# tmtlakmal/acme

Hardware: AMD Instinct MI355X
Metric: learner transitions/sec (sample+step) at batch 512, 1/2/4/8 MI355X (higher is better)
Workload: dtype f32 (2xf16 split planes, 3 MFMA terms); 1 GPU; dqn_nature_cnn_prioritized_replay (BASELINE configs[1]); global_batch=512, batch_per_gpu=512, replay_slots=1000000, replay_slots_per_gpu=1000000, obs=uint8[84,84,4], num_actions=18, sampler=prioritized(alpha=0.6), IS beta=0.2, prefetch_size=4, parallelism=dp1

## Files before the change

acme_amd/_lib.py:

```python

from __future__ import annotations

import ctypes
import os
import threading

import torch

_HERE = os.path.dirname(os.path.abspath(__file__))
LIB_PATH = os.environ.get("ACME_LIB_PATH") or os.path.join(_HERE, "libacme_hip.so")

ACME_OK = 0
ACME_ERR_INVALID = -1
ACME_ERR_HIP = -2
ACME_ERR_EMPTY = -3
ACME_ERR_OOM = -4

SEMANTICS_TF = 0
SEMANTICS_JAX = 1

MATMUL_F32 = 0
MATMUL_X6 = 1

MAX_FIELDS = 16
# ... 148 lines not shown
    "acme_set_matmul_engine": (c_i32, [c_i32]),
    "acme_matmul_engine": (c_i32, []),
    "acme_dense_forward": (c_i32, [c_vp, c_i64, c_i64, c_vp, c_vp, c_i64, c_i32, c_vp, c_vp]),
    "acme_dense_forward_staged": (c_i32, [c_vp, c_i64, c_i64, c_vp, c_vp, c_i64, c_i32, c_vp,
                                          c_i32, c_i32, c_i32, c_vp]),
    "acme_replay_create": (c_i32, [ctypes.POINTER(ReplayConfig), ctypes.POINTER(c_vp)]),
    "acme_replay_destroy": (c_i32, [c_vp]),
    "acme_replay_insert": (c_i32, [c_vp, ctypes.POINTER(c_vp), c_i64, c_vp, c_i32, c_vp, c_vp]),
    "acme_replay_stage_capacity": (c_i64, [c_vp]),
    "acme_replay_stage": (c_i32, [c_vp, c_i64, ctypes.POINTER(c_vp)]),
    "acme_replay_commit": (c_i32, [c_vp, c_i64, c_vp, c_vp, c_vp]),
    "acme_replay_sync_inserts": (c_i32, [c_vp]),
    "acme_host_register": (c_i32, [c_vp, c_i64]),
    "acme_event_create": (c_i32, [ctypes.POINTER(c_vp)]),
    "acme_event_destroy": (c_i32, [c_vp]),
    "acme_event_record": (c_i32, [c_vp, c_vp]),
    "acme_stream_wait_event": (c_i32, [c_vp, c_vp]),
    "acme_event_query": (c_i32, [c_vp]),
    "acme_event_synchronize": (c_i32, [c_vp]),
    "acme_host_unregister": (c_i32, [c_vp]),
    "acme_nstep_writer_create": (c_i32, [c_vp, c_i32, c_f32, c_i64, c_i64, c_i64, c_vp]),
    "acme_nstep_writer_destroy": (c_i32, [c_vp]),
    "acme_nstep_writer_start": (c_i32, [c_vp, c_vp]),
    "acme_nstep_writer_add": (c_i32, [c_vp, c_vp, c_f32, c_f32, c_vp, c_i32, c_f64]),
    "acme_nstep_writer_flush": (c_i32, [c_vp]),
    "acme_nstep_writer_reset": (c_i32, [c_vp]),
    "acme_nstep_writer_pending": (c_i64, [c_vp]),
    "acme_replay_fill_synthetic": (c_i32, [c_vp, c_i64, c_i32, c_i32, c_u64, c_vp]),
    "acme_replay_sample": (c_i32, [c_vp, c_i64, c_u64, c_vp, c_vp, c_vp, c_vp, c_vp, c_vp]),
    "acme_replay_gather": (c_i32, [c_vp, c_vp, c_i64, ctypes.POINTER(c_vp), c_vp]),
    "acme_replay_total": (c_i32, [c_vp, c_vp, c_vp]),
    "acme_replay_sample_share": (c_i32, [c_vp, c_i64, c_u64, c_f64, c_vp, c_vp, c_vp, c_vp, c_vp,
                                         ctypes.POINTER(c_vp), c_vp]),
    "acme_replay_sample_share_frames": (c_i32, [c_vp, c_i64, c_u64, c_f64, c_vp, c_vp, c_vp, c_vp,
                                                c_vp, ctypes.POINTER(c_vp), c_vp, c_vp]),
    "acme_replay_sample_gather": (c_i32, [c_vp, c_i64, c_u64, c_vp, c_vp, c_vp, c_vp, c_vp,
                                          ctypes.POINTER(c_vp), c_vp]),
    "acme_replay_sample_gather_frames": (c_i32, [c_vp, c_i64, c_u64, c_vp, c_vp, c_vp, c_vp,
                                                 c_vp, ctypes.POINTER(c_vp), c_vp, c_vp]),
    "acme_replay_pipe_open": (c_i32, [c_vp, ctypes.POINTER(c_i32)]),
    "acme_replay_pipe_close": (c_i32, [c_vp, c_i32]),
    "acme_replay_pipe_flush": (c_i32, [c_vp, c_i32]),
    "acme_replay_sample_gather_pipe": (c_i32, [c_vp, c_i32, c_i64, c_u64, c_vp, c_vp, c_vp, c_vp,
                                               c_vp, ctypes.POINTER(c_vp), c_vp]),
    "acme_r2d2_priorities": (c_i32, [c_vp, c_i32, c_i32, ctypes.c_double, c_vp, c_vp]),
    "acme_r2d2_importance_weights": (c_i32, [c_vp, c_i32, c_i64, ctypes.c_double, c_vp, c_vp]),
    "acme_frames_expand": (c_i32, [c_vp, c_i64, c_i64, c_i32, c_vp, c_i64, c_vp, c_vp]),
    "acme_replay_update_priorities": (c_i32, [c_vp, c_vp, c_vp, c_i64, c_vp]),
    "acme_replay_update_priorities_gated": (c_i32, [c_vp, c_vp, c_vp, c_i64, c_vp, c_vp]),
    "acme_replay_size": (c_i64, [c_vp]),
    "acme_replay_capacity": (c_i64, [c_vp]),
    "acme_replay_debug_leaves": (c_i32, [c_vp, ctypes.POINTER(c_vp), ctypes.POINTER(c_vp),
                                         ctypes.POINTER(c_vp)]),
    "acme_replay_storage": (c_i32, [c_vp, c_i32, ctypes.POINTER(c_vp)]),
    "acme_replay_inserted": (c_i64, [c_vp]),
    "acme_replay_restore": (c_i32, [c_vp, c_i64, c_vp]),
    "acme_dqn_create": (c_i32, [ctypes.POINTER(DQNConfig), ctypes.POINTER(c_vp)]),
    "acme_dqn_destroy": (c_i32, [c_vp]),
    "acme_dqn_num_params": (c_i64, [c_vp]),
    "acme_dqn_flat_size": (c_i64, [c_vp]),
    "acme_dqn_num_tensors": (c_i32, [c_vp]),
    "acme_dqn_tensor_info": (c_i32, [c_vp, c_i32, ctypes.POINTER(c_i64), ctypes.POINTER(c_i64),
                                     ctypes.POINTER(c_i32), ctypes.POINTER(c_i64),
                                     ctypes.POINTER(ctypes.c_char_p)]),
    "acme_dqn_bind": (c_i32, [c_vp, c_vp, c_vp, c_vp, c_vp, c_vp]),
    "acme_dqn_params_changed": (c_i32, [c_vp]),
    "acme_dqn_plane_overflow": (c_i32, [c_vp, ctypes.POINTER(c_i32), c_i32]),
    "acme_dqn_skipped_steps": (c_i64, [c_vp]),
    "acme_dqn_guard_state": (c_i32, [c_vp, ctypes.POINTER(c_i64)]),
    "acme_dqn_verdict_timeouts": (c_i32, [c_vp, ctypes.POINTER(c_i64)]),
    "acme_dqn_set_applied_steps": (c_i32, [c_vp, c_i64]),
    "acme_dqn_skip_word": (c_i32, [c_vp, ctypes.POINTER(c_vp)]),
    "acme_dqn_set_reissue": (c_i32, [c_vp, c_i32]),
    "acme_dqn_verdicts_issued": (c_i64, [c_vp]),
    "acme_dqn_step_verdict": (c_i32, [c_vp, c_i64, ctypes.POINTER(c_i32)]),
    "acme_dqn_set_data_parallel_gate": (c_i32, [c_vp, c_i32]),
    "acme_dqn_dense_grads_ready": (c_i32, [c_vp, c_vp]),
    "acme_dqn_dp_init": (c_i32, [c_vp, c_vp, c_i32]),
    "acme_dqn_dp_step": (c_i32, [c_vp, ctypes.POINTER(TransitionBatch), ctypes.POINTER(DQNOutputs),
                                 c_vp]),
    "acme_nccl_get_unique_id": (c_i32, [c_vp]),
    "acme_nccl_comm_init": (c_i32, [c_vp, c_i32, c_i32, ctypes.POINTER(c_vp)]),
    "acme_nccl_comm_destroy": (c_i32, [c_vp]),
    "acme_dqn_scale_state": (c_i32, [c_vp, c_vp, c_i32, ctypes.POINTER(c_i32)]),
    "acme_dqn_set_scale_state": (c_i32, [c_vp, c_vp, c_i32]),
    "acme_dqn_forward_backward": (c_i32, [c_vp, ctypes.POINTER(TransitionBatch),
                                          ctypes.POINTER(DQNOutputs), c_vp]),
    "acme_dqn_apply": (c_i32, [c_vp, c_vp]),
    "acme_dqn_forward_backward_stage": (c_i32, [c_vp, ctypes.POINTER(TransitionBatch),
                                                ctypes.POINTER(DQNOutputs), c_i32, c_vp]),
    "acme_dqn_grad_split": (c_i32, [c_vp, ctypes.POINTER(c_i64)]),
    "acme_dqn_step": (c_i32, [c_vp, ctypes.POINTER(TransitionBatch), ctypes.POINTER(DQNOutputs),
                              c_vp]),
    "acme_dqn_step_update": (c_i32, [c_vp, ctypes.POINTER(TransitionBatch),
                                     ctypes.POINTER(DQNOutputs), c_vp, c_vp, c_vp, c_vp]),
    "acme_dqn_q_values": (c_i32, [c_vp, c_vp, c_i64, c_i32, c_vp, c_vp]),
    "acme_dqn_num_steps": (c_i64, [c_vp]),
    "acme_dqn_debug_buffer": (c_i32, [c_vp, ctypes.c_char_p, ctypes.POINTER(c_vp),
                                      ctypes.POINTER(c_i64)]),
    "acme_dqn_set_num_steps": (c_i32, [c_vp, c_i64]),
    "acme_min_f64": (c_i32, [c_vp, c_i64, c_vp, c_vp]),
    "acme_r2d2_create": (c_i32, [ctypes.POINTER(R2D2Config), ctypes.POINTER(c_vp)]),
    "acme_r2d2_destroy": (c_i32, [c_vp]),
    "acme_r2d2_flat_size": (c_i64, [c_vp]),
    "acme_r2d2_num_tensors": (c_i32, [c_vp]),
    "acme_r2d2_tensor_info": (c_i32, [c_vp, c_i32, ctypes.POINTER(c_i64), ctypes.POINTER(c_i64),
                                      ctypes.POINTER(c_i32), ctypes.POINTER(c_i64),
                                      ctypes.POINTER(ctypes.c_char_p)]),
    "acme_r2d2_bind": (c_i32, [c_vp, c_vp, c_vp, c_vp, c_vp, c_vp]),
    "acme_r2d2_step": (c_i32, [c_vp, ctypes.POINTER(SequenceBatch), c_vp,
                               ctypes.POINTER(R2D2Outputs), c_vp]),
    "acme_r2d2_params_changed": (c_i32, [c_vp]),
    "acme_r2d2_scale_state": (c_i32, [c_vp, c_vp, c_i32, ctypes.POINTER(c_i32)]),
    "acme_r2d2_set_scale_state": (c_i32, [c_vp, c_vp, c_i32]),
    "acme_r2d2_skipped_steps": (c_i64, [c_vp]),
    "acme_r2d2_guard_state": (c_i32, [c_vp, ctypes.POINTER(c_i64)]),
    "acme_r2d2_skip_word": (c_vp, [c_vp]),
    "acme_r2d2_set_applied_steps": (c_i32, [c_vp, c_i64]),
    "acme_r2d2_num_steps": (c_i64, [c_vp]),
    "acme_r2d2_set_num_steps": (c_i32, [c_vp, c_i64]),
    "acme_r2d2_set_lstm_unroll": (c_i32, [c_vp, c_i32]),
    "acme_r2d2_debug_buffer": (c_i32, [c_vp, ctypes.c_char_p, ctypes.POINTER(c_vp),
                                       ctypes.POINTER(c_i64)]),
# ... 206 lines not shown
```

acme_amd/csrc/common.h:

```cpp
#pragma once

#include <hip/hip_runtime.h>

#include <cstdarg>
#include <cstdint>
#include <cstdio>

#include "../../include/acme_hip.h"

namespace acme {

void set_error(const char* fmt, ...);

int tune_variant(const char* key);
void tune_set(const char* key, int value);
int tune_generation();

hipError_t make_order_event(hipEvent_t* ev);

#define ACME_HIP_TRY(expr)                                                   \
  do {                                                                       \
    hipError_t _e = (expr);                                                  \
    if (_e != hipSuccess) {                                                  \
      ::acme::set_error("%s failed: %s (%s:%d)", #expr, hipGetErrorString(_e), \
                        __FILE__, __LINE__);                                 \
      return ACME_ERR_HIP;                                                   \
    }                                                                        \
  } while (0)

#define ACME_CHECK_ARG(cond, ...)                                            \
  do {                                                                       \
    if (!(cond)) {                                                           \
      ::acme::set_error(__VA_ARGS__);                                        \
      return ACME_ERR_INVALID;                                               \
    }                                                                        \
  } while (0)

#define ACME_LAUNCH_CHECK()                                                  \
  do {                                                                       \
    hipError_t _e = hipGetLastError();                                       \
    if (_e != hipSuccess) {                                                  \
      ::acme::set_error("kernel launch failed: %s (%s:%d)",                  \
                        hipGetErrorString(_e), __FILE__, __LINE__);          \
      return ACME_ERR_HIP;                                                   \
    }                                                                        \
  } while (0)

static inline hipStream_t as_stream(void* s) {
  return reinterpret_cast<hipStream_t>(s);
}

static inline int64_t ceil_div(int64_t a, int64_t b) { return (a + b - 1) / b; }

constexpr int kWave = 64;

__device__ __forceinline__ float wave_sum(float v) {
#pragma unroll
  for (int o = 32; o > 0; o >>= 1) v += __shfl_xor(v, o, 64);
  return v;
}
__device__ __forceinline__ float wave_max(float v) {
#pragma unroll
  for (int o = 32; o > 0; o >>= 1) v = fmaxf(v, __shfl_xor(v, o, 64));
  return v;
}

}
// ... 1 lines not shown
```

acme_amd/csrc/common.hip:

```cpp
#include "common.h"

#include <cstring>
#include <mutex>
#include <string>
#include <utility>
#include <vector>

namespace acme {

static thread_local char g_last_error[1024] = "";

void set_error(const char* fmt, ...) {
  va_list ap;
  va_start(ap, fmt);
  vsnprintf(g_last_error, sizeof(g_last_error), fmt, ap);
  va_end(ap);
}

namespace {
std::mutex g_tune_mu;
std::vector<std::pair<std::string, int>> g_tune;
int g_tune_gen = 0;
}

int tune_generation() {
  std::lock_guard<std::mutex> lock(g_tune_mu);
  return g_tune_gen;
}

int tune_variant(const char* key) {
  std::lock_guard<std::mutex> lock(g_tune_mu);
  for (auto& kv : g_tune)
    if (kv.first == key) return kv.second;
  const char* v = getenv((std::string("ACME_V_") + key).c_str());
  const int x = v ? atoi(v) : 0;
  g_tune.emplace_back(key, x);
  return x;
}

void tune_set(const char* key, int value) {
  std::lock_guard<std::mutex> lock(g_tune_mu);
  ++g_tune_gen;
  for (auto& kv : g_tune)
    if (kv.first == key) {
      kv.second = value;
      return;
    }
  g_tune.emplace_back(key, value);
}

namespace gemm {

static int g_engine = -1;

bool use_x6() {
  if (g_engine < 0) {
    const char* e = getenv("ACME_MATMUL");
    g_engine = (e && strcmp(e, "f32") == 0) ? ACME_MATMUL_F32 : ACME_MATMUL_X6;
  }
  return g_engine == ACME_MATMUL_X6;
}

}

hipError_t make_order_event(hipEvent_t* ev) {
  return hipEventCreateWithFlags(ev, hipEventDisableTiming | hipEventDisableSystemFence);
}

}

extern "C" {

int acme_set_matmul_engine(int32_t engine) {
  ACME_CHECK_ARG(engine == ACME_MATMUL_F32 || engine == ACME_MATMUL_X6, "unknown matmul engine %d",
                 engine);
  acme::gemm::g_engine = engine;
  return ACME_OK;
}

int32_t acme_matmul_engine(void) { return acme::gemm::use_x6() ? ACME_MATMUL_X6 : ACME_MATMUL_F32; }

const char* acme_last_error(void) { return acme::g_last_error; }

int acme_tune_set(const char* key, int32_t value) {
  ACME_CHECK_ARG(key, "null key");
  acme::tune_set(key, value);
  return ACME_OK;
}
// ... 47 lines not shown
```

acme_amd/csrc/dqn.hip:

```cpp
#include <hip/hip_runtime.h>

#include <algorithm>
#include <cmath>
#include <cstring>
#include <string>
#include <vector>

#include "common.h"
#include "conv.h"
#include "rescale.h"
#include "conv_p3.h"
#include "gemm.h"
#include "gemm_p3.h"
#include "gemm_x6.h"
#include "kernels.h"
#include "launch.h"
#include "learner_common.h"
#include "plane_guard.h"
#include "profiler.h"
#include "rccl_dyn.h"
#include "torso.h"

using namespace acme;
using namespace acme::conv;
using acme::gemm::launch_gemm;

namespace {

using torso::G1;
constexpr int kFlat = torso::kFlat;
constexpr int kHidden = 512;
constexpr int kObsBytes = 84 * 84 * 4;

struct Layer {
  int in = 0, out = 0;
  int w = -1, b = -1;
  bool relu = true;
};

}

struct acme_dqn : PlaneGuard {
  acme_dqn_config cfg;
  std::vector<Tensor> tensors;
  int64_t flat = 0, logical = 0;
  float *params = nullptr, *target = nullptr, *grads = nullptr, *m = nullptr, *v = nullptr;
  int64_t num_steps = 0;
  int t_c1w = -1, t_c1b, t_c2w, t_c2b, t_c3w, t_c3b, t_fcw, t_fcb, t_vw, t_vb, t_aw, t_ab;
  std::vector<Layer> layers;
  std::vector<void*> allocs;
  float *x1 = nullptr, *x2 = nullptr, *x3 = nullptr, *hid = nullptr;
  float *t1 = nullptr, *t2 = nullptr, *t3 = nullptr, *thid = nullptr;
  std::vector<float*> mlp_act, mlp_tact, mlp_dz;
  float *q_on = nullptr, *q_tg = nullptr;
  float *dzh = nullptr, *dz3 = nullptr, *dz2 = nullptr, *dz1 = nullptr;
  float* slab = nullptr;
  int64_t slab_floats = 0;
  bool stamps_on = false;
  uint64_t* stamps = nullptr;
  float* g = nullptr;
  int32_t* a_cache = nullptr;
  float* loss_tmp = nullptr;
  float* td_tmp = nullptr;
  double* prio_tmp = nullptr;
  bool p3_capable = false;
  bool planes_stale = true;
  bool last_p3 = false;
  uint16_t *wpl = nullptr, *tpl = nullptr;
  bool calibrating = false;
  int64_t fwd_batch = 0;
  uint16_t* frames = nullptr;
  torso::Frames cur_frames{nullptr};
  hipStream_t side = nullptr;
  hipEvent_t ev[4] = {nullptr, nullptr, nullptr, nullptr};
  float* slab2 = nullptr;
  bool fused_step = false;
  acme_replay* upd_replay = nullptr;
  const uint64_t* upd_keys = nullptr;
  hipEvent_t upd_after = nullptr;
  const double* upd_prio = nullptr;
  int upd_n = 0;
  bool slabs_pending = false;
  torso::WgradSlab wslabs[3];
  float* side_slab = nullptr;
  float* tslab = nullptr;
  bool target_dirty = true;
  torso::Plane x1p{}, x2p{}, x3p{}, t1p{}, t2p{}, t3p{}, dzhp{}, dz3p{}, dz2p{}, dz1p{};
  LossArgs pending_la{};
  bool loss_pending = false;
  bool head_deferred = false;
  int head_splits = 0;
  int64_t loss_nparts = 0;
  hipEvent_t ev_dense = nullptr;
  hipEvent_t dense_ev = nullptr;
  bool dense_on_side = false;
  void* dp_comm = nullptr;
  int dp_world = 0;
  hipStream_t dp_stream = nullptr;
  hipEvent_t dp_ev[4] = {nullptr, nullptr, nullptr, nullptr};
  double* dp_gmin = nullptr;
  double* loss_part = nullptr;
  bool single_stream = false;
  bool single_role = false;
  bool bk32 = false;
  bool frames_u8 = true;
  int64_t seq = 0;
  uint32_t* host_verdicts = nullptr;
  uint32_t verdict_seq = 0;
  bool sticky = false;
  bool dp_gate = false;
  int64_t dp_gate_index = -1;
  bool step_rescaled = false;
};

namespace {

enum {
  kScX1, kScX2, kScX3, kScT1, kScT2, kScT3, kScDzh, kScDz3, kScDz2, kScDz1,
  kScTransient,
  kScParams = kScTransient, kScTarget,
  kScCount
};
constexpr int64_t kParamAmaxPeriod = 8;
constexpr int kVerdictRing = 64;

int add_tensor(acme_dqn* l, const std::string& name, std::initializer_list<int64_t> shape) {
  const int t = acme::add_tensor<acme_dqn>(l, name, shape);
  l->logical += l->tensors[t].numel;
  return t;
}

inline torso::Plane WP(const acme_dqn* l, uint16_t* base, int t) {
  return torso::Plane{base + l->tensors[t].offset, l->flat,
                      l->scales + (base == l->tpl ? kScTarget : kScParams)};
}
int convert_frames(acme_dqn* l, const void* obs_a, const void* obs_b, int split, int rows,
                   hipStream_t st) {
  ACME_PROF("frames_f16", st, 0.0, 3.0 * (double)rows * kObsBytes);
  return launch_frames_f16(static_cast<const uint8_t*>(obs_a), static_cast<const uint8_t*>(obs_b),
                           split, rows, kObsBytes, l->frames, st);
}
bool use_p3(const acme_dqn* l) { return l->p3_capable && gemm::use_x6(); }
Gate step_gate(const acme_dqn* l) {
  Gate q;
  q.g = l->guard;
  q.par = (int)(l->seq & 1);
  if (l->dp_gate) q.dp = l->grads + l->dp_gate_index;
  return q;
}
hipStream_t side_stream(const acme_dqn* l) { return prof::enabled() ? nullptr : l->side; }

constexpr int kFcFwdSplits = 8;
constexpr int kHeadFwdSplits = 16;
constexpr int kHeadBwdSplits = 8;

int64_t slab_floats_needed(int B, int A) {
  return std::max<int64_t>({torso::wgrad_slab_floats(), (int64_t)kFcFwdSplits * 2 * B * 2 * kHidden,
// ... 117 lines not shown
    ACME_GEMM("mlp_fwd", 64, 64, 2, 2, 16, 1, p, 1);
  }
  return ACME_OK;
}

int mlp_forward(acme_dqn* l, const float* prm, const void* obs_a, const void* obs_b, int split,
                int rows, std::vector<float*>& act, float* q, hipStream_t st) {
  const int nl = (int)l->layers.size();
  for (int i = 0; i < nl; ++i) {
    const Layer& L = l->layers[i];
    float* y = i == nl - 1 ? q : act[i];
    int rc;
    if (i == 0) {
      rc = l->cfg.obs_dtype == ACME_OBS_U8_SCALED
               ? mlp_layer<InU8>(l, prm, L, obs_a, obs_b, split, rows, y, st)
               : mlp_layer<InF32>(l, prm, L, obs_a, obs_b, split, rows, y, st);
    } else {
      rc = mlp_layer<InF32>(l, prm, L, act[i - 1], act[i - 1], rows, rows, y, st);
    }
    if (rc != ACME_OK) return rc;
  }
  return ACME_OK;
}

RescaleJob step_rescale_job(acme_dqn* l, bool defer_r) {
  RescaleJob j;
  j.s = l->scales;
  j.nt = j.n = kScTransient;
  j.overflow = l->overflow;
  j.skip_lo = kScT1;
  j.skip_hi = kScT3 + 1;
  j.defer_r = defer_r ? 1 : 0;
  j.rg.g = l->guard;
  j.rg.mode = kRgStep;
  j.rg.gate = step_gate(l);
  j.rg.host_skipped = l->host_skipped;
  j.rg.host_verdicts = l->host_verdicts;
  j.rg.seq = l->verdict_seq++;
  j.rg.sticky = l->sticky ? 1 : 0;
  return j;
}

int priority_update_tail(void* ctx, hipStream_t st) {
  acme_dqn* l = static_cast<acme_dqn*>(ctx);
  acme_replay* r = l->upd_replay;
  if (!r || !l->upd_prio) return ACME_OK;
  l->upd_replay = nullptr;
  if (l->upd_after) ACME_HIP_TRY(hipStreamWaitEvent(st, l->upd_after, 0));
  const RescaleJob job = step_rescale_job(l, true);
  const int rc =
      replay_update_priorities_gated(r, l->upd_keys, l->upd_prio, l->upd_n, step_gate(l), st, &job);
  if (rc == ACME_OK) l->step_rescaled = true;
  return rc;
}

int nature_backward(acme_dqn* l, const void* o_tm1, int B, hipStream_t st_main,
                    bool join_dense) {
  hipStream_t st = st_main;
  const float* prm = l->params;
  float* gr = l->grads;
  const int A = l->cfg.num_actions;
  const bool p3 = use_p3(l);
  int rc;
  bool loss_sum = false;
  const LossArgs la = l->pending_la;
  if (p3 && l->loss_pending && l->head_deferred) {
    l->loss_pending = l->head_deferred = false;
    loss_sum = true;
    l->loss_nparts = B;
    ACME_PROF("head_loss_dz", st, 0.0, 4.0 * (double)2 * B * 2 * kHidden * (l->head_splits + 1));
    rc = launch_dqn_head_loss_dz(la, l->slab, l->head_splits, kHidden, P(l, prm, l->t_fcb),
                                 P(l, prm, l->t_vw), P(l, prm, l->t_vb), P(l, prm, l->t_aw),
                                 P(l, prm, l->t_ab), l->hid, l->dzhp.p, l->dzhp.stride,
                                 l->dzhp.sc, st);
    if (rc != ACME_OK) return rc;
  } else if (p3 && l->loss_pending) {
    l->loss_pending = false;
    loss_sum = la.loss_part != nullptr;
    l->loss_nparts = dqn_loss_head_dz_blocks(B, kHidden);
    ACME_PROF("loss_head_dz", st, 0.0, 0.0);
    rc = launch_dqn_loss_head_dz(la, l->hid, kHidden, P(l, prm, l->t_vw),
                                 P(l, prm, l->t_aw), l->dzhp.p, l->dzhp.stride, l->dzhp.sc, st);
    if (rc != ACME_OK) return rc;
  } else {
    ACME_PROF("head_dz", st, 0.0, 0.0);
    rc = p3 ? launch_head_dz_planes(l->hid, l->g, l->a_cache, B, kHidden, A, P(l, prm, l->t_vw),
                                    P(l, prm, l->t_aw), l->dzhp.p, l->dzhp.stride, l->dzhp.sc, st)
            : launch_duel_head_dz(l->hid, l->g, l->a_cache, B, kHidden, A, P(l, prm, l->t_vw),
                                  P(l, prm, l->t_aw), l->dzh, st);
    if (rc != ACME_OK) return rc;
  }
  const bool fork = p3 && side_stream(l);
  float* hslab = fork ? l->side_slab : l->slab;
  if (fork) {
    ACME_HIP_TRY(hipEventRecord(l->ev[2], st_main));
    ACME_HIP_TRY(hipStreamWaitEvent(l->side, l->ev[2], 0));
    st = l->side;
  }
  if (p3 && l->upd_replay && !l->calibrating) {
    l->upd_prio = la.prio;
    l->upd_n = B;
  }
  const bool sum_in_scatter = loss_sum;
  {
    DuelHeadWgrad p;
    p.M = 2 * kHidden; p.N = A + 1; p.K = B; p.k_chunk = chunk_for(B, kHeadBwdSplits);
// ... 93 lines not shown
        ACME_GEMM("mlp_dgrad", 64, 64, 2, 2, 16, 1, p, 1);
      } else {
        DenseDgrad<false> p;
        p.M = B; p.N = L.in; p.K = L.out; p.k_chunk = L.out;
        p.dz = dz; p.w = P(l, prm, L.w); p.xprev = l->mlp_act[i - 1]; p.ldx = L.in;
        p.dx = l->mlp_dz[i - 1];
        ACME_GEMM("mlp_dgrad", 64, 64, 2, 2, 16, 1, p, 1);
      }
    }
  }
  return ACME_OK;
}

int sync_planes(acme_dqn* l, hipStream_t st) {
  if (!l->p3_capable || !l->planes_stale) return ACME_OK;
  int rc = launch_split_planes(l->params, l->flat, l->wpl, l->flat, l->scales + kScParams, st,
                               l->overflow, 1);
  if (rc == ACME_OK)
    rc = launch_split_planes(l->target, l->flat, l->tpl, l->flat, l->scales + kScTarget, st,
                             l->overflow, 1);
  if (rc == ACME_OK) l->planes_stale = false;
  return rc;
}

int reset_scales(acme_dqn* l) {
  return scales_init(l, kScCount, [l](int i) {
    return i >= kScT1 && i <= kScT3 ? &l->guard->tt
           : i >= kScTransient     ? &l->guard->prm
                                   : &l->guard->on;
  });
}

}

extern "C" {

int acme_dqn_create(const acme_dqn_config* cfg, acme_dqn** out) {
  ACME_CHECK_ARG(cfg && out, "null argument");
  ACME_CHECK_ARG(cfg->num_actions >= 1 && cfg->num_actions <= 63, "num_actions must be in [1, 63]");
  ACME_CHECK_ARG(cfg->max_batch >= 1 && cfg->max_batch <= 65536, "max_batch must be in [1, 65536]");
  ACME_CHECK_ARG(cfg->network == ACME_NET_NATURE_DQN || cfg->network == ACME_NET_MLP,
                 "unknown network kind %d", cfg->network);
  ACME_CHECK_ARG(cfg->obs_dtype == ACME_OBS_U8_SCALED || cfg->obs_dtype == ACME_OBS_F32,
                 "unknown observation dtype %d", cfg->obs_dtype);
  ACME_CHECK_ARG(cfg->huber_loss_parameter >= 0.f, "quadratic_linear_boundary must be >= 0.");
  ACME_CHECK_ARG(cfg->target_update_period >= 1, "target_update_period must be >= 1");
  ACME_CHECK_ARG(cfg->semantics == ACME_SEMANTICS_TF || cfg->semantics == ACME_SEMANTICS_JAX,
                 "unknown learner semantics %d", cfg->semantics);
  acme_dqn* l = new acme_dqn();
  l->cfg = *cfg;
  l->single_stream = tune_variant("SIDE") == 1;
  l->single_role = tune_variant("WSN") == 1;
  l->bk32 = tune_variant("BK32") == 1;
  l->stamps_on = tune_variant("STAMPS") == 1;
  const int A = cfg->num_actions;
  const int B = cfg->max_batch;
  int rc = ACME_OK;
  auto fail = [&](int code) {
    acme_dqn_destroy(l);
    return code;
  };
  if ((rc = guard_create(l)) != ACME_OK) return fail(rc);
  if (hipHostMalloc(reinterpret_cast<void**>(&l->host_verdicts), kVerdictRing * sizeof(uint32_t),
                    hipHostMallocCoherent | hipHostMallocMapped) != hipSuccess)
    return fail((set_error("step guard allocation failed"), ACME_ERR_HIP));
  for (int i = 0; i < kVerdictRing; ++i) l->host_verdicts[i] = 0xFFFFFFFFu;
  if (cfg->network == ACME_NET_NATURE_DQN) {
    l->t_c1w = add_tensor(l, "atari_torso/conv2_d/w", {8, 8, 4, 32});
    l->t_c1b = add_tensor(l, "atari_torso/conv2_d/b", {32});
    l->t_c2w = add_tensor(l, "atari_torso/conv2_d_1/w", {4, 4, 32, 64});
    l->t_c2b = add_tensor(l, "atari_torso/conv2_d_1/b", {64});
    l->t_c3w = add_tensor(l, "atari_torso/conv2_d_2/w", {3, 3, 64, 64});
    l->t_c3b = add_tensor(l, "atari_torso/conv2_d_2/b", {64});
    l->t_fcw = add_tensor(l, "duelling_q_network/hidden/w", {kFlat, 2 * kHidden});
    l->t_fcb = add_tensor(l, "duelling_q_network/hidden/b", {2 * kHidden});
    l->t_vw = add_tensor(l, "duelling_q_network/mlp/linear_1/w", {kHidden, 1});
    l->t_vb = add_tensor(l, "duelling_q_network/mlp/linear_1/b", {1});
    l->t_aw = add_tensor(l, "duelling_q_network/mlp_1/linear_1/w", {kHidden, A});
    l->t_ab = add_tensor(l, "duelling_q_network/mlp_1/linear_1/b", {A});
    const int R2 = 2 * B;
    if ((rc = dev_alloc(l, &l->x1, (int64_t)R2 * G1::OPIX * G1::CO)) ||
        (rc = dev_alloc(l, &l->x2, (int64_t)R2 * kFlat)) ||
        (rc = dev_alloc(l, &l->x3, (int64_t)R2 * kFlat)) ||
        (rc = dev_alloc(l, &l->hid, (int64_t)R2 * 2 * kHidden)) ||
        (rc = dev_alloc(l, &l->t1, (int64_t)B * G1::OPIX * G1::CO)) ||
        (rc = dev_alloc(l, &l->t2, (int64_t)B * kFlat)) ||
        (rc = dev_alloc(l, &l->t3, (int64_t)B * kFlat)) ||
        (rc = dev_alloc(l, &l->thid, (int64_t)B * 2 * kHidden)) ||
        (rc = dev_alloc(l, &l->dzh, (int64_t)B * 2 * kHidden)) ||
        (rc = dev_alloc(l, &l->dz3, (int64_t)B * kFlat)) ||
        (rc = dev_alloc(l, &l->dz2, (int64_t)B * kFlat)) ||
        (rc = dev_alloc(l, &l->dz1, (int64_t)B * G1::OPIX * G1::CO)))
      return fail(rc);
    l->slab_floats = slab_floats_needed(B, A);
    if (cfg->obs_dtype == ACME_OBS_U8_SCALED && (int64_t)R2 * kObsBytes * 2 < (int64_t)INT32_MAX) {
      l->p3_capable = true;
      const int64_t fl = l->flat;
      if ((rc = reset_scales(l)) ||
          (rc = dev_alloc(l, &l->wpl, gemm::kPlanes * fl)) ||
          (rc = dev_alloc(l, &l->tpl, gemm::kPlanes * fl)) ||
          (rc = dev_alloc(l, &l->frames, (int64_t)R2 * kObsBytes)) ||
          (rc = plane_alloc(l, &l->x1p, (int64_t)R2 * torso::kX1, kScX1)) ||
          (rc = plane_alloc(l, &l->x2p, (int64_t)R2 * kFlat, kScX2)) ||
          (rc = plane_alloc(l, &l->x3p, (int64_t)R2 * kFlat, kScX3)) ||
          (rc = plane_alloc(l, &l->t1p, (int64_t)B * torso::kX1, kScT1)) ||
          (rc = plane_alloc(l, &l->t2p, (int64_t)B * kFlat, kScT2)) ||
// ... 109 lines not shown
  l->grads = grads;
  l->m = adam_m;
  l->v = adam_v;
  l->planes_stale = true;
  l->scales_ok = false;
  return ACME_OK;
}

int acme_dqn_params_changed(acme_dqn* l) {
  ACME_CHECK_ARG(l, "null learner");
  l->planes_stale = true;
  l->scales_ok = false;
  l->target_dirty = true;
  return ACME_OK;
}

int acme_dqn_scale_state(const acme_dqn* l, float* out, int32_t capacity, int32_t* count) {
  return scale_state(l, out, capacity, count);
}

int acme_dqn_set_scale_state(acme_dqn* l, const float* in, int32_t count) {
  const int rc = set_scale_state(l, in, count);
  if (rc == ACME_OK) l->target_dirty = true;
  return rc;
}

int acme_dqn_plane_overflow(acme_dqn* l, int32_t* overflow, int32_t reset) {
  return plane_overflow(l, overflow, reset);
}

int64_t acme_dqn_skipped_steps(const acme_dqn* l) { return skipped_steps(l); }

int acme_dqn_guard_state(acme_dqn* l, int64_t* out4) {
  ACME_CHECK_ARG(l && out4 && l->guard, "null argument");
  StepGuard g;
  if (int rc = read_guard(l, &g)) return rc;
  out4[0] = g.applied;
  out4[1] = g.skipped;
  out4[2] = g.last;
  out4[3] = g.qv;
  return ACME_OK;
}

int acme_dqn_verdict_timeouts(acme_dqn* l, int64_t* out) {
  ACME_CHECK_ARG(l && out, "null argument");
  *out = 0;
  if (!l->guard) return ACME_OK;
  StepGuard g;
  if (int rc = read_guard(l, &g)) return rc;
  *out = g.vtimeout;
  return ACME_OK;
}

int acme_dqn_set_reissue(acme_dqn* l, int32_t enable) {
  ACME_CHECK_ARG(l, "null learner");
  l->sticky = enable != 0 && l->p3_capable;
  return ACME_OK;
}

int64_t acme_dqn_verdicts_issued(const acme_dqn* l) { return l ? (int64_t)l->verdict_seq : 0; }

int acme_dqn_step_verdict(const acme_dqn* l, int64_t seq, int32_t* state) {
  ACME_CHECK_ARG(l && state && seq >= 0, "bad argument");
  *state = -1;
  if (!l->host_verdicts || seq >= (int64_t)l->verdict_seq) return ACME_OK;
  ACME_CHECK_ARG(seq + kVerdictRing >= (int64_t)l->verdict_seq,
                 "verdict %lld is older than the ring's %d", (long long)seq, kVerdictRing);
  const uint32_t v =
      __atomic_load_n(l->host_verdicts + (seq & (kVerdictRing - 1)), __ATOMIC_ACQUIRE);
  if ((v >> 1) == ((uint32_t)seq & 0x7fffffffu)) *state = (int32_t)(v & 1u);
  return ACME_OK;
}

int acme_dqn_set_applied_steps(acme_dqn* l, int64_t n) {
  ACME_CHECK_ARG(l && l->guard && n >= 0, "bad argument");
  return set_applied(l, n);
}

int acme_dqn_skip_word(const acme_dqn* l, const uint32_t** out) {
  ACME_CHECK_ARG(l && out, "null argument");
  *out = l->p3_capable ? &l->guard->last : nullptr;
  return ACME_OK;
}

int acme_dqn_set_data_parallel_gate(acme_dqn* l, int32_t enable) {
  ACME_CHECK_ARG(l, "null learner");
  if (enable && l->cfg.network == ACME_NET_NATURE_DQN && l->p3_capable) {
    const Tensor& t = l->tensors[l->t_c1b];
    ACME_CHECK_ARG(align64(t.offset + t.numel) > t.offset + t.numel, "no padding word for the gate");
    l->dp_gate_index = t.offset + t.numel;
    l->dp_gate = true;
  } else {
    l->dp_gate = false;
  }
  return ACME_OK;
}

int64_t acme_dqn_num_steps(const acme_dqn* l) { return l ? l->num_steps : 0; }
int acme_dqn_set_num_steps(acme_dqn* l, int64_t n) {
  ACME_CHECK_ARG(l && n >= 0, "bad argument");
  l->num_steps = n;
  return ACME_OK;
}

int acme_dqn_debug_buffer(const acme_dqn* l, const char* name, const float** out,
                          int64_t* count) {
// ... 85 lines not shown
constexpr int kCalibrationPasses = 4;
static int calibrate_scales(acme_dqn* l, const acme_transition_batch* batch, hipStream_t st) {
  acme_transition_batch cb = *batch;
  cb.global_min_probability = nullptr;
  l->calibrating = true;
  int rc = ACME_OK;
  for (int pass = 0; pass < kCalibrationPasses && rc == ACME_OK; ++pass) {
    rc = forward_backward_stage(l, &cb, nullptr, 2, st, false);
    if (rc == ACME_OK) rc = forward_backward_stage(l, &cb, nullptr, 3, st, false);
    if (rc == ACME_OK) rc = forward_backward_stage(l, &cb, nullptr, 1, st, false);
    if (rc == ACME_OK)
      rc = launch_plane_rescale(l->scales, kScTransient, kScTransient, -1, -1, l->overflow, st);
  }
  l->calibrating = false;
  if (rc != ACME_OK) return rc;
  return calibration_done(l, st);
}

static int forward_backward_stage(acme_dqn* l, const acme_transition_batch* batch,
                                  const acme_dqn_outputs* out, int32_t stage, void* stream,
                                  bool join_dense) {
  ACME_CHECK_ARG(l && batch && l->params, "null argument or unbound learner");
  ACME_CHECK_ARG(stage >= 0 && stage <= 4, "stage must be 0, 1, 2, 3 or 4");
  ACME_CHECK_ARG(batch->o_tm1 && batch->a_tm1 && batch->r_t && batch->d_t && batch->o_t &&
                     batch->probabilities,
                 "transition batch has null fields");
  ACME_CHECK_ARG(batch->batch >= 1 && batch->batch <= l->cfg.max_batch,
                 "batch %lld outside [1, max_batch=%d]", (long long)batch->batch, l->cfg.max_batch);
  hipStream_t st = as_stream(stream);
  const int B = (int)batch->batch;
  const bool nature = l->cfg.network == ACME_NET_NATURE_DQN;
  if (stage == 1) {
    if (!nature) return ACME_OK;
    if (use_p3(l)) {
      torso::Grads g{Pm(l, l->grads, l->t_c1w), Pm(l, l->grads, l->t_c1b),
                     Pm(l, l->grads, l->t_c2w), Pm(l, l->grads, l->t_c2b),
                     Pm(l, l->grads, l->t_c3w), Pm(l, l->grads, l->t_c3b)};
      torso::PWeights w{WP(l, l->wpl, l->t_c1w), WP(l, l->wpl, l->t_c2w),
                        WP(l, l->wpl, l->t_c3w), P(l, l->params, l->t_c1b),
                        P(l, l->params, l->t_c2b), P(l, l->params, l->t_c3b)};
      torso::Side sd;
      sd.single_role = l->single_role;
      sd.bk32 = l->bk32;
      sd.conv1_single = true;
      if (side_stream(l)) {
        sd.side = l->side;
        sd.slab = l->side_slab;
        for (int i = 0; i < 3; ++i) sd.e[i] = l->ev[i];
      }
      l->slabs_pending = false;
      if (l->upd_replay && l->upd_prio && !l->calibrating) {
        sd.tail = priority_update_tail;
        sd.tail_ctx = l;
      }
      if (l->fused_step && !l->calibrating && l->slab2) {
        sd.slab = l->side_slab;
        sd.slab2 = l->slab2;
        sd.defer = l->wslabs;
        l->slabs_pending = true;
      }
      int rc = torso::backward_p3(w, g, l->cur_frames, B,
                                  torso::PActs{l->x1p, l->x2p, l->x3p}, l->dz3p, l->dz2p, l->dz1p,
                                  l->slab, st, sd);
      if (rc == ACME_OK && l->dp_gate && !l->calibrating) {
        Gate local = step_gate(l);
        local.dp = nullptr;
        rc = launch_gate_publish(local, l->grads + l->dp_gate_index, st, l->scales,
                                 kScTransient, kScT1, kScT3 + 1);
      }
      return rc;
    }
    torso::Grads g{Pm(l, l->grads, l->t_c1w), Pm(l, l->grads, l->t_c1b), Pm(l, l->grads, l->t_c2w),
                   Pm(l, l->grads, l->t_c2b), Pm(l, l->grads, l->t_c3w), Pm(l, l->grads, l->t_c3b)};
    return torso::backward(torso_weights(l, l->params), g,
                           l->cfg.obs_dtype == ACME_OBS_U8_SCALED, batch->o_tm1, B,
                           torso::Acts{l->x1, l->x2, l->x3}, l->dz3, l->dz2, l->dz1, l->slab, st);
  }
  const int A = l->cfg.num_actions;
  int rc;
  if (stage == 3 || stage == 4) {
    ACME_CHECK_ARG(l->fwd_batch == (int64_t)B, "stage %d needs the stage-2 forward of this batch",
                   stage);
    l->fwd_batch = 0;
    return loss_and_dense_backward(l, batch, out, st, join_dense && stage == 3);
  }
  l->last_p3 = nature && use_p3(l);
  if (l->last_p3) {
    const bool u8 = !batch->obs_f16 && l->frames_u8 &&
                    ((reinterpret_cast<uintptr_t>(batch->o_tm1) |
                      reinterpret_cast<uintptr_t>(batch->o_t)) & 15) == 0;
    const bool quiet =
        !l->planes_stale && l->scales_ok && (batch->obs_f16 || u8) && !l->calibrating;
    if ((rc = sync_planes(l, st)) != ACME_OK) return rc;
    if (!l->scales_ok && !l->calibrating && (rc = calibrate_scales(l, batch, st)) != ACME_OK)
      return rc;
    l->last_p3 = true;
    hipStream_t tst = st;
    hipStream_t side = side_stream(l);
    if (!batch->obs_f16 && !u8 &&
        (rc = convert_frames(l, batch->o_tm1, batch->o_t, B, 2 * B, st)) != ACME_OK)
      return rc;
    const torso::Frames fwd_frames =
        u8 ? torso::Frames{batch->o_tm1, true, batch->o_t, B}
           : torso::Frames{batch->obs_f16 ? static_cast<const void*>(batch->obs_f16)
                                          : static_cast<const void*>(l->frames)};
    l->cur_frames = fwd_frames;
// ... 338 lines not shown
```

acme_amd/csrc/gemm_p3.h:

```cpp
#pragma once

#include <hip/hip_runtime.h>

#include <cstdint>
#include <type_traits>

#include "gemm.h"
#include "gemm_x6.h"

namespace acme {
namespace gemm {

struct BlockPlace {
  int m0, n0, z;
};
template <int BM, int BN>
__device__ __forceinline__ BlockPlace place_block(int M, int N, int n_major) {
  const int tiles = gridDim.x;
  const int total = tiles * gridDim.z;
  const int orig = blockIdx.x + tiles * blockIdx.z;
  const int xcd = orig & 7, q = total >> 3, r = total & 7;
  const int L = (xcd < r ? xcd * (q + 1) : r * (q + 1) + (xcd - r) * q) + (orig >> 3);
  const int z = L / tiles, t = L - z * tiles;
  const int tiles_m = (M + BM - 1) / BM, tiles_n = (N + BN - 1) / BN;
  int mt, nt;
  if (n_major) {
    nt = t / tiles_m;
    mt = t - nt * tiles_m;
  } else {
    mt = t / tiles_n;
    nt = t - mt * tiles_n;
  }
  return BlockPlace{mt * BM, nt * BN, z};
}
template <class P>
__device__ __forceinline__ P z_select_at(const P& p, int z) {
  if constexpr (HasZClass<P>::value) return p.for_z(z);
  else return p;
}

using u32x4 = __attribute__((ext_vector_type(4))) uint32_t;
using i16x4 = __attribute__((ext_vector_type(4))) short;
using f16x8 = __attribute__((ext_vector_type(8))) _Float16;

__device__ __forceinline__ u32x4 zero_u4() { return u32x4{0u, 0u, 0u, 0u}; }

constexpr uint32_t kOOB = 0x80000000u;

constexpr int kPlanes = 2;

constexpr int kAmaxSlots = 64;
struct PScale {
  float w, r, wi, rl;
  uint32_t* flag;
  uint32_t pad1[26];
  struct Slot {
    uint32_t v;
    uint32_t pad[31];
  } slot[kAmaxSlots];
};
static_assert(sizeof(PScale) == 128 * (1 + kAmaxSlots), "one 128-B line per amax slot");
__device__ __forceinline__ float read_scale(const PScale* s) { return s ? s->r : 1.f; }

struct PlaneSrc {
  const uint16_t* p;
  int64_t stride;
  int32_t bytes;
  const PScale* sc = nullptr;
};
__device__ __forceinline__ __amdgpu_buffer_rsrc_t plane_rsrc(const PlaneSrc& s, int pl) {
  return __builtin_amdgcn_make_buffer_rsrc(const_cast<uint16_t*>(s.p + pl * s.stride), (short)0,
                                           s.bytes, 0x00020000);
}
__device__ __forceinline__ float result_scale(const PlaneSrc& a, const PlaneSrc& b) {
  return read_scale(a.sc) * read_scale(b.sc);
}

__device__ __forceinline__ void split2_bits(float y, uint16_t& h, uint16_t& l) {
  const _Float16 hb = (_Float16)y;
  const _Float16 lb = (_Float16)(y - (float)hb);
  h = __builtin_bit_cast(uint16_t, hb);
  l = __builtin_bit_cast(uint16_t, lb);
}
__device__ __forceinline__ float f16_bits_to_f32(uint16_t b) {
  return (float)__builtin_bit_cast(_Float16, b);
}
// ... 375 lines not shown
                                                  int wave, int wm, int wn, int lane, int split,
                                                  f32x16 (&acc)[MT][NTL], f32x16 (&cs)[NCS],
                                                  bool do_colsum,
                                                  const typename EpiPre<P>::type* pre = nullptr) {
    static_assert(HasStore8<P>::value, "plane problems store 8 columns at a time");
    const int r = lane & 31, h = lane >> 5;
    typename EpiPre<P>::type pl{};
    if constexpr (EpiPre<P>::has) pl = pre ? *pre : p.pre(n0 + wn * TN + epi_col(lane));
    constexpr int PITCH = TN + 4;
    float* cw = reinterpret_cast<float*>(smem) + wave * 32 * PITCH;
    constexpr int CHUNKS = 32 * TN / 8;
    float amx = 0.f;
#pragma unroll
    for (int i = 0; i < MT; ++i) {
#pragma unroll
      for (int j = 0; j < NTL; ++j)
#pragma unroll
        for (int v = 0; v < 16; ++v)
          cw[((v & 3) + 8 * (v >> 2) + 4 * h) * PITCH + j * 32 + r] = acc[i][j][v];
      __syncthreads();
#pragma unroll
      for (int c = lane; c < CHUNKS; c += 64) {
        const int row = c / (TN / 8), col = 8 * (c % (TN / 8));
        const int m = m0 + wm * TM + i * 32 + row;
        const int n = n0 + wn * TN + col;
        const f32x4 lo = *reinterpret_cast<const f32x4*>(cw + row * PITCH + col);
        const f32x4 hi = *reinterpret_cast<const f32x4*>(cw + row * PITCH + col + 4);
        const float v8[8] = {lo[0], lo[1], lo[2], lo[3], hi[0], hi[1], hi[2], hi[3]};
        if constexpr (EpiPre<P>::has) {
          if (m < p.M && n < p.N) amx = amax_max(amx, p.store8p(m, n, v8, split, pl));
        } else {
          if (m < p.M && n < p.N) amx = amax_max(amx, p.store8(m, n, v8, split));
        }
      }
      __syncthreads();
    }
    if constexpr (HasAmax<P>::value) {
      if constexpr (EpiPre<P>::has) amax_commit_pre(p.amax_sc(), amx, pl.w, pl.flag);
      else amax_commit(p.amax_sc(), amx);
    }
    if constexpr (kColSum) {
      if (do_colsum && h == 0) {
#pragma unroll
        for (int j = 0; j < NTL; ++j) {
          const int n = n0 + wn * TN + j * 32 + r;
          if (n < p.N) p.store_colsum(n, cs[j][0], split);
        }
      }
    }
  }
};

template <int BM, int BN, int WM, int WN, int BK, bool DEEP, class P>
__global__ void __launch_bounds__(64 * WM * WN) gemm_p3_kernel(const P p_in, int n_major) {
  using C = P3Core<BM, BN, WM, WN, BK, P>;
  using PA = typename C::PA;
  using PB = typename C::PB;
  constexpr int NT = C::NT, NPA = C::NPA, NPB = C::NPB, STAGE = C::STAGE;
  const BlockPlace bp = place_block<BM, BN>(p_in.M, p_in.N, n_major);
  const P p = z_select_at(p_in, bp.z);
  extern __shared__ __attribute__((aligned(16))) uint8_t smem[];

  const int tid = threadIdx.x;
  const int lane = tid & 63, wave = tid >> 6;
  const int wm = wave / WN, wn = wave % WN;
  const int m0 = bp.m0, n0 = bp.n0;
  const int split = HasZClass<P>::value ? 0 : bp.z;
  const int kbeg = split * p.k_chunk;
  int kend = kbeg + p.k_chunk;
  if (kend > p.K) kend = p.K;
  const int nk = kend > kbeg ? (kend - kbeg + BK - 1) / BK : 0;

  typename P::ARow arow[PA::PER_THREAD];
  typename P::BRow brow[PB::PER_THREAD];
#pragma unroll
  for (int i = 0; i < PA::PER_THREAD; ++i)
    arow[i] = p.a_row(m0 + (PA::owns(tid + i * NT) ? PA::row_of(tid + i * NT) : 0));
#pragma unroll
  for (int i = 0; i < PB::PER_THREAD; ++i)
    brow[i] = p.b_row(n0 + (PB::owns(tid + i * NT) ? PB::row_of(tid + i * NT) : 0));

  __amdgpu_buffer_rsrc_t srcA[NPA], srcB[NPB];
#pragma unroll
  for (int pl = 0; pl < NPA; ++pl) srcA[pl] = plane_rsrc(p.a_src, pl);
#pragma unroll
  for (int pl = 0; pl < NPB; ++pl) srcB[pl] = plane_rsrc(p.b_src, pl);

  constexpr int SETS = DEEP ? 2 : 1;
  u32x4 ra[SETS][PA::PER_THREAD][NPA], rb[SETS][PB::PER_THREAD][NPB];
  auto fetch = [&](auto S, int k0) {
    constexpr int set = decltype(S)::value;
#pragma unroll
    for (int i = 0; i < PA::PER_THREAD; ++i) {
      const int u = tid + i * NT;
      const int kk = PA::kk_of(u);
      const uint32_t off = (PA::owns(u) && k0 + kk < kend) ? p.a_off(arow[i], k0, kk) : kOOB;
#pragma unroll
      for (int pl = 0; pl < NPA; ++pl) {
        ra[set][i][pl] = load_a_unit<P>(srcA[pl], off);
      }
    }
#pragma unroll
    for (int i = 0; i < PB::PER_THREAD; ++i) {
      const int u = tid + i * NT;
      const int kk = PB::kk_of(u);
      const uint32_t off = (PB::owns(u) && k0 + kk < kend) ? p.b_off(brow[i], k0, kk) : kOOB;
#pragma unroll
      for (int pl = 0; pl < NPB; ++pl)
        rb[set][i][pl] =
            __builtin_bit_cast(u32x4, __builtin_amdgcn_raw_buffer_load_b128(srcB[pl], off, 0, 0));
    }
  };
  auto stash = [&](auto S, int buf) {
    constexpr int set = decltype(S)::value;
// ... 23 lines not shown
  acc.zero();
  const bool do_colsum = C::kColSum && m0 == 0 && wm == 0;
  auto compute = [&](int buf) {
    const uint8_t* sa = smem + buf * STAGE;
    C::mma(sa, sa + PA::BYTES, wm, wn, lane, acc, do_colsum);
  };

  using S0 = std::integral_constant<int, 0>;
  using S1 = std::integral_constant<int, 1>;
  if constexpr (DEEP) {
    if (nk > 0) {
      fetch(S0{}, kbeg);
      stash(S0{}, 0);
    }
    if (nk > 1) fetch(S1{}, kbeg + BK);
    __syncthreads();
    auto iter = [&](auto S, int kt) {
      constexpr int set = decltype(S)::value;
      using Other = std::integral_constant<int, set ^ 1>;
      if constexpr (BK == 32) {
        const uint8_t* sa = smem + set * STAGE;
        C::template mma<0, 1>(sa, sa + PA::BYTES, wm, wn, lane, acc, do_colsum);
        stash(Other{}, set ^ 1);
        fetch(S, kbeg + (kt + 2) * BK);
        C::template mma<1, 2>(sa, sa + PA::BYTES, wm, wn, lane, acc, do_colsum);
      } else {
        stash(Other{}, set ^ 1);
        fetch(S, kbeg + (kt + 2) * BK);
        compute(set);
      }
      __syncthreads();
    };
    int kt = 0;
    for (; kt + 1 < nk; kt += 2) {
      iter(S0{}, kt);
      iter(S1{}, kt + 1);
    }
    if (kt < nk) iter(S0{}, kt);
  } else {
    if (nk > 0) {
      fetch(S0{}, kbeg);
      stash(S0{}, 0);
    }
    __syncthreads();
    for (int kt = 0; kt < nk; ++kt) {
      const bool more = kt + 1 < nk;
      if (more) fetch(S0{}, kbeg + (kt + 1) * BK);
      compute(kt & 1);
      if (more) stash(S0{}, (kt + 1) & 1);
      __syncthreads();
    }
  }
  C::epilogue(p, smem, m0, n0, wave, wm, wn, lane, split, acc, do_colsum);
}

template <int BM, int BN, int WM, int WN, int BK, int STAGES, class P>
__global__ void __launch_bounds__(64 * WM * WN) gemm_p3g_kernel(const P p_in, int n_major) {
#if defined(__HIP_DEVICE_COMPILE__)
  using C = P3Core<BM, BN, WM, WN, BK, P>;
  using PA = typename C::PA;
  using PB = typename C::PB;
  constexpr int NW = WM * WN, NPA = C::NPA, NPB = C::NPB, STAGE = C::STAGE;
  constexpr int PWA = (PA::BLOCKS + NW - 1) / NW, PWB = (PB::BLOCKS + NW - 1) / NW;
  static_assert(!AU8<P>::value, "LDS-DMA copies bytes as they are: no uint8 A operand");
  constexpr int D = PWA * NPA + PWB * NPB;
  static_assert(STAGES >= 2 && STAGES <= 4, "2..4 LDS stages");
  static_assert((STAGES - 2) * D <= 63, "vmcnt range");
  const BlockPlace bp = place_block<BM, BN>(p_in.M, p_in.N, n_major);
  const P p = z_select_at(p_in, bp.z);
  extern __shared__ __attribute__((aligned(16))) uint8_t smem[];
  uint8_t* scratch = smem + STAGES * STAGE;

  const int tid = threadIdx.x;
  const int lane = tid & 63, wave = __builtin_amdgcn_readfirstlane(tid >> 6);
  const int wm = wave / WN, wn = wave % WN;
  const int m0 = bp.m0, n0 = bp.n0;
  const int split = HasZClass<P>::value ? 0 : bp.z;
  const int kbeg = split * p.k_chunk;
  int kend = kbeg + p.k_chunk;
  if (kend > p.K) kend = p.K;
  const int nk = kend > kbeg ? (kend - kbeg + BK - 1) / BK : 0;

  typename P::ARow arow[PWA];
  typename P::BRow brow[PWB];
  int akk[PWA], bkk[PWB];
#pragma unroll
  for (int j = 0; j < PWA; ++j) {
    const int b = wave + NW * j;
    const int u = 64 * (b < PA::BLOCKS ? b : 0) + lane;
    arow[j] = p.a_row(m0 + PA::slot_row(u));
    akk[j] = PA::slot_kk(u);
  }
#pragma unroll
  for (int j = 0; j < PWB; ++j) {
    const int b = wave + NW * j;
    const int u = 64 * (b < PB::BLOCKS ? b : 0) + lane;
    brow[j] = p.b_row(n0 + PB::slot_row(u));
    bkk[j] = PB::slot_kk(u);
  }
  __amdgpu_buffer_rsrc_t srcA[NPA], srcB[NPB];
#pragma unroll
  for (int pl = 0; pl < NPA; ++pl) srcA[pl] = plane_rsrc(p.a_src, pl);
#pragma unroll
  for (int pl = 0; pl < NPB; ++pl) srcB[pl] = plane_rsrc(p.b_src, pl);

  typedef __attribute__((address_space(3))) void lds_void;
// ... 208 lines not shown
      C::mma(sa, sa + PA::BYTES, wm, wn, lane, acc, do_colsum);
      rbuf = rbuf == RING - 1 ? 0 : rbuf + 1;
      __syncthreads();
    }
  }
  if constexpr (HasStamps<P>::value)
    if (stamp) st_t2 = __builtin_amdgcn_s_memtime();
  C::epilogue(p, smem, m0, n0, wave, wm, wn, lane, split, acc, do_colsum);
  if constexpr (HasStamps<P>::value) {
    if (stamp) {
      const uint64_t t3 = __builtin_amdgcn_s_memtime(), rt1 = __builtin_amdgcn_s_memrealtime();
      uint64_t* o = p.stamps + 8 * ((int64_t)blockIdx.z * gridDim.x + blockIdx.x);
      o[0] = st_rt0;
      o[1] = rt1;
      o[2] = st_t0;
      o[3] = st_t1;
      o[4] = st_t2;
      o[5] = t3;
    }
  }
}

template <class P>
inline int p3_n_major(const P& p) {
  return (int64_t)p.N * P::B_PLANES > (int64_t)p.M * P::A_PLANES ? 1 : 0;
}

template <class P>
constexpr double p3_peak_tflops() {
  return 2500.0 / (double)p3_nterms<P::A_PLANES, P::B_PLANES>();
}

template <class Kern>
inline hipError_t p3_set_lds(Kern* k, int lds) {
  if (lds <= 65536) return hipSuccess;
  return hipFuncSetAttribute(reinterpret_cast<const void*>(k),
                             hipFuncAttributeMaxDynamicSharedMemorySize, lds);
}

template <int BM, int BN, int WM, int WN, int BK, bool DEEP = true, class P>
inline hipError_t launch_gemm_p3(const P& p, int splits, hipStream_t st) {
  using C = P3Core<BM, BN, WM, WN, BK, P>;
  constexpr int STAGES_BYTES = 2 * C::STAGE;
  constexpr int LDS = STAGES_BYTES > C::EPI_BYTES ? STAGES_BYTES : C::EPI_BYTES;
  static_assert(LDS <= 160 * 1024, "two stages must fit the 160-KiB LDS of a CU");
  static hipError_t attr = p3_set_lds(&gemm_p3_kernel<BM, BN, WM, WN, BK, DEEP, P>, LDS);
  if (attr != hipSuccess) return attr;
  const int tiles = ((p.N + BN - 1) / BN) * ((p.M + BM - 1) / BM);
  hipLaunchKernelGGL((gemm_p3_kernel<BM, BN, WM, WN, BK, DEEP, P>), dim3(tiles, 1, splits),
                     dim3(C::NT), LDS, st, p, p3_n_major(p));
  return hipGetLastError();
}

template <int BM, int BN, int WM, int WN, int BK, bool PIPE = false, class P>
inline hipError_t launch_gemm_p3ws(const P& p, int splits, hipStream_t st) {
  using C = P3Core<BM, BN, WM, WN, BK, P>;
  constexpr int RING_BYTES = 3 * C::STAGE;
  constexpr int LDS = RING_BYTES > C::EPI_BYTES ? RING_BYTES : C::EPI_BYTES;
  static_assert(LDS <= 160 * 1024, "three stages must fit the 160-KiB LDS of a CU");
  static hipError_t attr = p3_set_lds(&gemm_p3ws_kernel<BM, BN, WM, WN, BK, PIPE, P>, LDS);
  if (attr != hipSuccess) return attr;
  const int tiles = ((p.N + BN - 1) / BN) * ((p.M + BM - 1) / BM);
  hipLaunchKernelGGL((gemm_p3ws_kernel<BM, BN, WM, WN, BK, PIPE, P>), dim3(tiles, 1, splits),
                     dim3(2 * C::NT), LDS, st, p, p3_n_major(p));
  return hipGetLastError();
}

template <int BM, int BN, int WM, int WN, int BK, int STAGES, class P>
inline hipError_t launch_gemm_p3g(const P& p, int splits, hipStream_t st) {
  using C = P3Core<BM, BN, WM, WN, BK, P>;
  constexpr int RING = STAGES * C::STAGE + 1024;
  constexpr int LDS = RING > C::EPI_BYTES ? RING : C::EPI_BYTES;
  static_assert(LDS <= 160 * 1024, "the stage ring must fit the 160-KiB LDS of a CU");
  static hipError_t attr = p3_set_lds(&gemm_p3g_kernel<BM, BN, WM, WN, BK, STAGES, P>, LDS);
  if (attr != hipSuccess) return attr;
  const int tiles = ((p.N + BN - 1) / BN) * ((p.M + BM - 1) / BM);
  hipLaunchKernelGGL((gemm_p3g_kernel<BM, BN, WM, WN, BK, STAGES, P>), dim3(tiles, 1, splits),
                     dim3(C::NT), LDS, st, p, p3_n_major(p));
  return hipGetLastError();
}

}
}
```

acme_amd/csrc/replay.hip:

```cpp
#include <hip/hip_runtime.h>

#include <algorithm>
#include <cmath>
#include <cstring>
#include <condition_variable>
#include <mutex>
#include <thread>
#include <vector>

#include "common.h"
#include "detmath.h"
#include "kernels.h"
#include "profiler.h"
#include "rescale.h"

namespace acme {
uint64_t* g_update_stamps = nullptr;
}

using namespace acme;

constexpr int kStageChunks = 4;
constexpr int64_t kStageBytes = 32ll << 20;
constexpr int kMaxReaders = 8;
constexpr int kMaxPipes = 8;

struct acme_replay {
  acme_replay_config cfg;
  int nlevels = 0;
  int64_t level_size[8] = {};
  double* levels[8] = {};
  double* raw_prio = nullptr;
  uint64_t* keys = nullptr;
  int32_t* winner = nullptr;
  uint32_t* upd_done = nullptr;
  int64_t* upd_slots = nullptr;
  int32_t* upd_valid = nullptr;
  int64_t upd_cap = 0;
  uint8_t* fields[ACME_MAX_FIELDS] = {};
  int64_t inserted = 0;
  std::mutex mu;
  hipStream_t side = nullptr;
  hipStream_t upload = nullptr;
  hipEvent_t insert_event = nullptr;
  uint64_t insert_seq = 0;
  int64_t stage_items = 0;
  int64_t stage_off[ACME_MAX_FIELDS + 3] = {};
  uint8_t* stage[kStageChunks] = {};
  uint8_t* stage_dev[kStageChunks] = {};
  hipEvent_t stage_up[kStageChunks] = {};
  hipEvent_t stage_done[kStageChunks] = {};
  bool stage_used[kStageChunks] = {};
  int stage_next = 0;
  int staged = -1;
  int64_t staged_n = 0;
  std::thread::id staged_by;
  std::condition_variable stage_cv;
  struct Reader {
    hipStream_t s;
    hipEvent_t ev;
    uint64_t waited;
    bool dirty;
  } readers[kMaxReaders] = {};
  int nreaders = 0;
  std::mutex order_mu;
  struct Pipe {
    bool open, pending;
    hipEvent_t ev;
    hipStream_t st;
    int64_t batch;
    const int64_t* slots;
    void* out[ACME_MAX_FIELDS];
  } pipes[kMaxPipes] = {};
};

namespace {

__device__ __forceinline__ double wave_scan64(double x) {
  const int lane = threadIdx.x & 63;
#pragma unroll
  for (int d = 1; d < 64; d <<= 1) {
    double y = __shfl_up(x, d, 64);
    if (lane >= d) x = y + x;
  }
  return x;
}

template <int Ctrl>
__device__ __forceinline__ double dpp_f64(double x) {
  const uint64_t u = __builtin_bit_cast(uint64_t, x);
  const int lo = __builtin_amdgcn_mov_dpp((int)(uint32_t)u, Ctrl, 0xf, 0xf, false);
  const int hi = __builtin_amdgcn_mov_dpp((int)(uint32_t)(u >> 32), Ctrl, 0xf, 0xf, false);
  return __builtin_bit_cast(double, ((uint64_t)(uint32_t)hi << 32) | (uint32_t)lo);
}
__device__ __forceinline__ double wave_total64(double x) {
  x = x + dpp_f64<0xB1>(x);
  x = x + dpp_f64<0x4E>(x);
  x = x + dpp_f64<0x141>(x);
  x = x + dpp_f64<0x140>(x);
  const uint64_t u = __builtin_bit_cast(uint64_t, x);
  const int lo = __builtin_amdgcn_ds_swizzle((int)(uint32_t)u, 0x401F);
  const int hi = __builtin_amdgcn_ds_swizzle((int)(uint32_t)(u >> 32), 0x401F);
  x = x + __builtin_bit_cast(double, ((uint64_t)(uint32_t)hi << 32) | (uint32_t)lo);
  const uint64_t v = __builtin_bit_cast(uint64_t, x);
  const uint32_t a0 = __builtin_amdgcn_readlane((int)(uint32_t)v, 31);
  const uint32_t a1 = __builtin_amdgcn_readlane((int)(uint32_t)(v >> 32), 31);
  const uint32_t b0 = __builtin_amdgcn_readlane((int)(uint32_t)v, 63);
  const uint32_t b1 = __builtin_amdgcn_readlane((int)(uint32_t)(v >> 32), 63);
  return __builtin_bit_cast(double, ((uint64_t)a1 << 32) | a0) +
         __builtin_bit_cast(double, ((uint64_t)b1 << 32) | b0);
}

__device__ __forceinline__ int select_child(double v, double s, double t) {
  const uint64_t le = __ballot(s <= t);
  const uint64_t nz = __ballot(v > 0.0);
  int idx = __popcll(le);
  const int last = nz ? 63 - __clzll(nz) : 0;
  if (idx > last) idx = last;
  return idx;
}

constexpr int kTopComputed = 16;
struct TreeView {
  const double* level[8];
  int nlevels;
  int top_nodes = 0;
};

__device__ __forceinline__ double top_entry(const double* const* level, int nlevels,
                                            int top_nodes) {
  const int lane = threadIdx.x & 63;
  if (top_nodes <= 0) return level[nlevels - 1][lane];
  const double* c = level[nlevels - 2];
  double ch[kTopComputed];
#pragma unroll
  for (int g = 0; g < kTopComputed; ++g) ch[g] = g < top_nodes ? c[g * 64 + lane] : 0.0;
  double v = 0.0;
#pragma unroll
  for (int g = 0; g < kTopComputed; ++g) {
    if (g >= top_nodes) break;
    const double t = wave_total64(ch[g]);
    if (lane == g) v = t;
  }
  return v;
}

__device__ __forceinline__ bool draw_prioritized(const TreeView& tree, double u,
                                                 int64_t* slot_out, double* prob_out) {
  const int lane = threadIdx.x & 63;
  int64_t node = 0;
  double t = 0.0, total = 0.0, leaf_value = 0.0;
  const int top = tree.nlevels - 1;
  double ch[kTopComputed];
  for (int l = top; l >= 0; --l) {
    const int64_t base = node * 64;
    double v;
    if (l == top) {
      if (tree.top_nodes > 0) {
        const double* c = tree.level[top - 1];
#pragma unroll
        for (int g = 0; g < kTopComputed; ++g) ch[g] = g < tree.top_nodes ? c[g * 64 + lane] : 0.0;
        v = 0.0;
#pragma unroll
        for (int g = 0; g < kTopComputed; ++g) {
          if (g >= tree.top_nodes) break;
// ... 384 lines not shown
    int shift) {
  const int lane = threadIdx.x & 63;
  const int64_t j = (int64_t)blockIdx.x * (blockDim.x >> 6) + (threadIdx.x >> 6);
  if (j >= count) return;
  int64_t node;
  if (slots) {
    if (valid && !valid[j]) return;
    node = slots[j] >> shift;
  } else {
    node = node_begin + j;
  }
  const double v = child[node * 64 + lane];
  const double s = wave_total64(v);
  if (lane == 63) parent[node] = s;
}

__global__ void prio_resolve_kernel(const uint64_t* __restrict__ upd_keys, int64_t n,
                                    const uint64_t* __restrict__ keys, int64_t capacity,
                                    int64_t* __restrict__ out_slots,
                                    int32_t* __restrict__ valid, int32_t* __restrict__ winner) {
  const int64_t j = (int64_t)blockIdx.x * blockDim.x + threadIdx.x;
  if (j >= n) return;
  const uint64_t k = upd_keys[j];
  const int64_t slot = (int64_t)(k % (uint64_t)capacity);
  const int ok = keys[slot] == k;
  out_slots[j] = slot;
  valid[j] = ok;
  if (ok) atomicMax(&winner[slot], (int32_t)j);
}

__global__ void prio_write_kernel(const double* __restrict__ prios, int64_t n,
                                  const int64_t* __restrict__ slots,
                                  const int32_t* __restrict__ valid,
                                  const int32_t* __restrict__ winner, double alpha,
                                  double* __restrict__ raw_prio, double* __restrict__ leaves,
                                  const Gate gate) {
  const int64_t j = (int64_t)blockIdx.x * blockDim.x + threadIdx.x;
  if (j >= n || !valid[j] || gate_skip(gate)) return;
  const int64_t slot = slots[j];
  if (winner[slot] != (int32_t)j) return;
  const double p = prios[j];
  raw_prio[slot] = p;
  leaves[slot] = det_pow_priority(p, alpha);
}

__global__ void prio_reset_kernel(const int64_t* __restrict__ slots,
                                  const int32_t* __restrict__ valid, int64_t n,
                                  int32_t* __restrict__ winner) {
  const int64_t j = (int64_t)blockIdx.x * blockDim.x + threadIdx.x;
  if (j >= n || !valid[j]) return;
  winner[slots[j]] = -1;
}

constexpr int kFusedUpdateMax = 4096;
constexpr int kFusedUpdateBlocks = 256;
constexpr int kUpdPairs = 32;
struct FusedUpdateArgs {
  const uint64_t* upd_keys;
  const double* prios;
  int n;
  int64_t capacity;
  const uint64_t* keys;
  double alpha;
  double* raw_prio;
  double* level[8];
  int64_t top_nodes;
  int top_computed;
  int nlevels;
  uint32_t* done;
  Gate gate;
  RescaleJob job;
  uint64_t* stamps = nullptr;
};
__device__ __forceinline__ bool wait_verdict_skip(StepGuard* g, uint32_t seq, uint32_t first) {
  __shared__ uint32_t s_v;
  if (threadIdx.x == 0) {
    uint32_t v = first;
    for (int it = 0; it < (1 << 22) && (v >> 1) != (seq & 0x7fffffffu); ++it) {
      __builtin_amdgcn_s_sleep(2);
      v = __hip_atomic_load(&g->vseq, __ATOMIC_RELAXED, __HIP_MEMORY_SCOPE_AGENT);
    }
    const bool got = (v >> 1) == (seq & 0x7fffffffu);
    if (!got) atomicAdd(&g->vtimeout, 1u);
    s_v = got ? (v & 1u) : 1u;
  }
  __syncthreads();
  return s_v != 0u;
}
__device__ __forceinline__ void lds_barrier() {
  __builtin_amdgcn_fence(__ATOMIC_RELEASE, "workgroup", "local");
  __builtin_amdgcn_s_barrier();
  __builtin_amdgcn_fence(__ATOMIC_ACQUIRE, "workgroup", "local");
}
__device__ __forceinline__ void store_shared_level(double* p, double v) {
  __hip_atomic_store(p, v, __ATOMIC_RELAXED, __HIP_MEMORY_SCOPE_AGENT);
}
template <int R>
__global__ void __launch_bounds__(256) prio_update_fused_kernel(FusedUpdateArgs a) {
  static_assert(R * 256 <= kFusedUpdateMax, "update capacity");
  __shared__ int64_t s_slot[R * 256];
  __shared__ int s_len, s_np, s_ovf, s_last;
  __shared__ double s_ch[kUpdPairs][64];
  __shared__ int64_t s_node[kUpdPairs];
  __shared__ int s_lvl[kUpdPairs];
  __shared__ int64_t s_nk[kUpdPairs];
  __shared__ double s_val[kUpdPairs];
  const int first = a.job.s ? 1 : 0;
  auto stamp = [&](int ph) {
    if (a.stamps && threadIdx.x == 0)
      a.stamps[8 * (int64_t)blockIdx.x + ph] = __builtin_amdgcn_s_memrealtime();
  };
  stamp(0);
  if (a.job.s && blockIdx.x == 0) {
    rescale_block(a.job);
    stamp(1);
    return;
  }
  const bool verdict = a.job.s && a.job.rg.g && a.job.rg.mode == kRgStep;
  const int tid = threadIdx.x, nt = blockDim.x;
  const int lane = tid & 63, wave = tid >> 6, nw = nt >> 6;
  const int G = kFusedUpdateBlocks, bid = (int)blockIdx.x - first;
  const int h = a.nlevels >= 2 ? a.nlevels - 2 : 0;
  bool skip = !verdict && gate_skip(a.gate);
  if (tid == 0) s_len = 0;
  __syncthreads();
  uint64_t kv[R];
  double pr[R];
  int64_t sl[R];
  int my_e[R];
#pragma unroll
  for (int i = 0; i < R; ++i) {
    my_e[i] = -1;
    kv[i] = 0;
    pr[i] = 0.0;
    sl[i] = 0;
  }
  if (!skip) {
#pragma unroll
    for (int i = 0; i < R; ++i) {
      if (i * nt >= a.n) break;
      const int j = tid + i * nt;
      const int jc = j < a.n ? j : a.n - 1;
      kv[i] = a.upd_keys[jc];
      pr[i] = a.prios[jc];
    }
#pragma unroll
    for (int i = 0; i < R; ++i) {
      if (i * nt >= a.n) break;
      const int j = tid + i * nt;
      const int64_t slot = (int64_t)(kv[i] % (uint64_t)a.capacity);
      if (j < a.n && (int)((slot >> (6 * h)) % G) == bid) {
        const int e = atomicAdd(&s_len, 1);
        s_slot[e] = slot;
        my_e[i] = e;
        sl[i] = slot;
      }
    }
  }
  __syncthreads();
  stamp(1);
  const int len = s_len;
  if (len > 0) {
    if (tid == 0) {
      s_np = 0;
      s_ovf = 0;
    }
    __syncthreads();
    for (int idx = tid; idx < h * len; idx += nt) {
      const int l = 1 + idx / len, e = idx - (l - 1) * len;
      const int64_t node = s_slot[e] >> (6 * l);
      bool first = true;
      for (int f = 0; f < e && first; ++f) first = (s_slot[f] >> (6 * l)) != node;
      if (!first) continue;
      const int q = atomicAdd(&s_np, 1);
      if (q < kUpdPairs) {
        s_lvl[q] = l;
        s_node[q] = node;
        s_nk[q] = (node << 3) | l;
      } else {
        s_ovf = 1;
      }
    }
    __syncthreads();
    if (tid == 0 && s_np > kUpdPairs) s_np = kUpdPairs;
    __syncthreads();
    stamp(2);
    const int np = s_np;
    const bool pre = !s_ovf;
    uint64_t kt[R];
#pragma unroll
    for (int i = 0; i < R; ++i) {
      if (i * nt >= a.n) break;
      kt[i] = my_e[i] >= 0 ? a.keys[sl[i]] : 0;
    }
    if (pre) {
      for (int q = wave; q < np; q += nw)
        s_ch[q][lane] = a.level[s_lvl[q] - 1][s_node[q] * 64 + lane];
    }
    double leafv[R];
#pragma unroll
    for (int i = 0; i < R; ++i) {
      if (i * nt >= a.n) break;
      leafv[i] = 0.0;
      if (my_e[i] >= 0) leafv[i] = det_pow_priority(pr[i], a.alpha);
    }
#pragma unroll
    for (int i = 0; i < R; ++i) {
      if (i * nt >= a.n) break;
      if (my_e[i] >= 0)
        s_slot[my_e[i]] = (sl[i] << 13) | ((kt[i] == kv[i] ? 1 : 0) << 12) | (tid + i * nt);
    }
    __syncthreads();
    stamp(4);
    uint32_t vfirst = 0;
    if (verdict && tid == 0)
      vfirst = __hip_atomic_load(&a.job.rg.g->vseq, __ATOMIC_RELAXED, __HIP_MEMORY_SCOPE_AGENT);
    bool winv[R];
#pragma unroll
    for (int i = 0; i < R; ++i) winv[i] = false;
#pragma unroll
    for (int i = 0; i < R; ++i) {
      if (i * nt >= a.n) break;
      const int e = my_e[i];
      bool win = e >= 0 && kt[i] == kv[i];
      const int j = tid + i * nt;
      const int64_t me = (sl[i] << 1) | 1;
#pragma unroll 4
      for (int f = 0; f < len; ++f) {
        const int64_t x = s_slot[f];
        if ((x >> 12) == me && (int)(x & 4095) > j) win = false;
      }
      winv[i] = win;
    }
    if (pre) {
#pragma unroll
      for (int i = 0; i < R; ++i) {
        if (i * nt >= a.n) break;
        if (!winv[i]) continue;
        const int64_t k1 = ((sl[i] >> 6) << 3) | 1;
#pragma unroll 4
        for (int q = 0; q < np; ++q)
          if (s_nk[q] == k1) s_ch[q][sl[i] & 63] = leafv[i];
      }
    }
    lds_barrier();
    if (pre) {
      for (int l = 1; l <= h; ++l) {
        for (int q = wave; q < np; q += nw) {
          if (s_lvl[q] != l) continue;
          const double v = wave_total64(s_ch[q][lane]);
          if (lane == 63) s_val[q] = v;
        }
        lds_barrier();
        if (tid < np && s_lvl[tid] == l) {
          const int64_t kp = ((s_node[tid] >> 6) << 3) | (l + 1);
#pragma unroll 4
          for (int q = 0; q < np; ++q)
            if (s_nk[q] == kp) s_ch[q][s_node[tid] & 63] = s_val[tid];
        }
        lds_barrier();
      }
    }
    stamp(7);
    if (verdict) skip = wait_verdict_skip(a.job.rg.g, a.job.rg.seq, vfirst);
    stamp(3);
    if (!skip) {
#pragma unroll
      for (int i = 0; i < R; ++i) {
        if (i * nt >= a.n) break;
        if (!winv[i]) continue;
        a.raw_prio[sl[i]] = pr[i];
        if (h == 0 && !a.top_computed) store_shared_level(a.level[0] + sl[i], leafv[i]);
        else a.level[0][sl[i]] = leafv[i];
      }
      if (pre) {
        for (int q = tid; q < np; q += nt) {
          const int l = s_lvl[q];
          if (l == h && !a.top_computed) store_shared_level(a.level[l] + s_node[q], s_val[q]);
          else a.level[l][s_node[q]] = s_val[q];
        }
      } else {
        __syncthreads();
        for (int l = 1; l <= h; ++l) {
          for (int e = wave; e < len; e += nw) {
            const int64_t node = (s_slot[e] >> 13) >> (6 * l);
            const double v = wave_total64(a.level[l - 1][node * 64 + lane]);
            if (lane == 63) {
              if (l == h && !a.top_computed) store_shared_level(a.level[l] + node, v);
              else a.level[l][node] = v;
            }
          }
          __syncthreads();
        }
      }
      stamp(5);
    }
  }
  stamp(6);
  if (a.nlevels < 2 || a.top_computed) return;
  __builtin_amdgcn_fence(__ATOMIC_RELEASE, "agent");
  __syncthreads();
  if (tid == 0)
    s_last = __hip_atomic_fetch_add(a.done, 1u, __ATOMIC_ACQ_REL, __HIP_MEMORY_SCOPE_AGENT) ==
             (uint32_t)(G - 1);
  __syncthreads();
  if (!s_last) return;
  __builtin_amdgcn_fence(__ATOMIC_ACQUIRE, "agent");
  const int top = a.nlevels - 1;
  for (int64_t node = wave; node < a.top_nodes; node += nw) {
    const double c = __hip_atomic_load(a.level[top - 1] + node * 64 + lane, __ATOMIC_RELAXED,
                                       __HIP_MEMORY_SCOPE_AGENT);
    const double v = wave_total64(c);
    if (lane == 63) a.level[top][node] = v;
  }
  if (tid == 0) __hip_atomic_store(a.done, 0u, __ATOMIC_RELAXED, __HIP_MEMORY_SCOPE_AGENT);
}



__global__ void fill_i32_kernel(int32_t* p, int64_t n, int32_t v) {
  const int64_t i = (int64_t)blockIdx.x * blockDim.x + threadIdx.x;
  if (i < n) p[i] = v;
}

__device__ __forceinline__ u32x4 fill_rand(uint64_t seed, uint64_t item, uint32_t chunk,
                                          uint32_t field) {
  u32x4 c = {chunk, (uint32_t)item, (uint32_t)(item >> 32) ^ (field << 24), kFillTag};
  return philox4x32_10(c, (uint32_t)seed, (uint32_t)(seed >> 32));
}

__global__ void __launch_bounds__(256) fill_bytes_kernel(uint8_t* __restrict__ field,
                                                         int64_t row_bytes, int64_t capacity,
                                                         int64_t first_key, int64_t n,
                                                         uint64_t seed, uint32_t field_id) {
  const int64_t nvec = row_bytes >> 4;
  const int64_t total = n * nvec;
  for (int64_t i = (int64_t)blockIdx.x * blockDim.x + threadIdx.x; i < total;
       i += (int64_t)gridDim.x * blockDim.x) {
    const int64_t item = i / nvec, v = i - item * nvec;
    const int64_t key = first_key + item;
    const int64_t slot = key % capacity;
    const u32x4 r = fill_rand(seed, (uint64_t)key, (uint32_t)v, field_id);
    uint4 w = {r.x, r.y, r.z, r.w};
    reinterpret_cast<uint4*>(field + slot * row_bytes)[v] = w;
  }
}

__global__ void fill_f32_normal_kernel(float* __restrict__ field, int64_t row_floats,
                                       int64_t capacity, int64_t first_key, int64_t n,
                                       uint64_t seed, uint32_t field_id, float lo, float hi,
                                       int uniform) {
  const int64_t total = n * row_floats;
  for (int64_t i = (int64_t)blockIdx.x * blockDim.x + threadIdx.x; i < total;
       i += (int64_t)gridDim.x * blockDim.x) {
    const int64_t item = i / row_floats, c = i - item * row_floats;
    const int64_t key = first_key + item;
    const u32x4 r = fill_rand(seed, (uint64_t)key, (uint32_t)c, field_id);
    const double u1 = u01_53(r.x, r.y), u2 = u01_53(r.z, r.w);
    float x;
    if (uniform) {
      x = lo + (hi - lo) * (float)u1;
    } else {
      x = (float)(sqrt(-2.0 * log(1.0 - u1)) * cos(6.283185307179586 * u2));
    }
    field[(key % capacity) * row_floats + c] = x;
  }
}

__global__ void fill_scalars_kernel(int32_t* __restrict__ action, float* __restrict__ reward,
                                    float* __restrict__ discount, int reward_uniform,
                                    float p_zero_discount, float nonzero_discount,
// ... 365 lines not shown
  (void)hipMemset(r->keys, 0xFF, cfg->capacity * sizeof(uint64_t));
  fill_i32_kernel<<<(unsigned)ceil_div(cfg->capacity, 256), 256>>>(r->winner, cfg->capacity, -1);
  for (int f = 0; f < cfg->num_fields; ++f) {
    if (hipMalloc(&r->fields[f], cfg->capacity * cfg->field_bytes[f]) != hipSuccess)
      return fail("field storage");
  }
  if (hipDeviceSynchronize() != hipSuccess) return fail("init sync");
  *out = r;
  return ACME_OK;
}

int acme_replay_destroy(acme_replay* r) {
  if (!r) return ACME_OK;
  (void)hipDeviceSynchronize();
  for (int l = 0; l < 8; ++l)
    if (r->levels[l]) (void)hipFree(r->levels[l]);
  if (r->raw_prio) (void)hipFree(r->raw_prio);
  if (r->keys) (void)hipFree(r->keys);
  if (r->winner) (void)hipFree(r->winner);
  if (r->upd_done) (void)hipFree(r->upd_done);
  if (r->upd_slots) (void)hipFree(r->upd_slots);
  if (r->upd_valid) (void)hipFree(r->upd_valid);
  for (int f = 0; f < ACME_MAX_FIELDS; ++f)
    if (r->fields[f]) (void)hipFree(r->fields[f]);
  for (int c = 0; c < kStageChunks; ++c) {
    if (r->stage[c]) (void)hipHostFree(r->stage[c]);
    if (r->stage_dev[c]) (void)hipFree(r->stage_dev[c]);
    if (r->stage_done[c]) (void)hipEventDestroy(r->stage_done[c]);
    if (r->stage_up[c]) (void)hipEventDestroy(r->stage_up[c]);
  }
  for (int i = 0; i < r->nreaders; ++i) (void)hipEventDestroy(r->readers[i].ev);
  for (auto& p : r->pipes)
    if (p.ev) (void)hipEventDestroy(p.ev);
  if (r->insert_event) (void)hipEventDestroy(r->insert_event);
  if (r->side) (void)hipStreamDestroy(r->side);
  if (r->upload) (void)hipStreamDestroy(r->upload);
  delete r;
  return ACME_OK;
}

int64_t acme_replay_size(const acme_replay* r) {
  if (!r) return 0;
  return std::min(r->inserted, r->cfg.capacity);
}

int64_t acme_replay_capacity(const acme_replay* r) { return r ? r->cfg.capacity : 0; }

int acme_replay_debug_leaves(const acme_replay* r, const double** leaf_values,
                             const double** raw_priorities, const uint64_t** keys) {
  ACME_CHECK_ARG(r, "null replay");
  if (leaf_values) *leaf_values = r->levels[0];
  if (raw_priorities) *raw_priorities = r->raw_prio;
  if (keys) *keys = r->keys;
  return ACME_OK;
}

int acme_replay_storage(acme_replay* r, int32_t field, void** out) {
  ACME_CHECK_ARG(r && out, "null argument");
  ACME_CHECK_ARG(field >= 0 && field < r->cfg.num_fields, "field %d out of range", field);
  {
    std::lock_guard<std::mutex> lock(r->mu);
    const int rc = flush_pipes(r, true);
    if (rc != ACME_OK) return rc;
  }
  *out = r->fields[field];
  return ACME_OK;
}

int64_t acme_replay_inserted(const acme_replay* r) { return r ? r->inserted : 0; }

int acme_replay_restore(acme_replay* r, int64_t inserted, void* stream) {
  ACME_CHECK_ARG(r, "null replay");
  ACME_CHECK_ARG(inserted >= 0, "negative insert count");
  std::lock_guard<std::mutex> lock(r->mu);
  hipStream_t st = as_stream(stream);
  int rc = flush_pipes(r, true);
  if (rc != ACME_OK) return rc;
  rc = order_after_inserts(r, st);
  if (rc != ACME_OK) return rc;
  const int64_t C = r->cfg.capacity, live = std::min(inserted, C);
  const int64_t n = r->level_size[0];
  restore_leaves_kernel<<<(unsigned)ceil_div(n, 256), 256, 0, st>>>(
      r->raw_prio, r->levels[0], live, n, r->cfg.sampler == ACME_SAMPLER_PRIORITIZED,
      r->cfg.priority_exponent);
  ACME_LAUNCH_CHECK();
  for (int l = 1; l < r->nlevels; ++l) {
    const int64_t count = r->level_size[l - 1] / 64;
    level_update_kernel<<<(unsigned)ceil_div(count, 4), 256, 0, st>>>(
        r->levels[l - 1], r->levels[l], 0, count, nullptr, nullptr, 0);
    ACME_LAUNCH_CHECK();
  }
  std::lock_guard<std::mutex> olock(r->order_mu);
  r->inserted = inserted;
  return ACME_OK;
}

int64_t acme_replay_stage_capacity(acme_replay* r) {
  if (!r) return 0;
  std::lock_guard<std::mutex> lock(r->mu);
  if (ensure_insert_path(r) != ACME_OK) return 0;
  return r->stage_items;
}

int acme_replay_stage(acme_replay* r, int64_t n, void** field_ptrs) {
  ACME_CHECK_ARG(r && field_ptrs, "null argument");
  std::unique_lock<std::mutex> lock(r->mu);
// ... 492 lines not shown
  const int32_t nvec = pair ? (int32_t)(r->cfg.field_bytes[f0] / 16) : 0;
  bool ride = p.pending && pair && p.st == st && p.slots != slots;
  for (int f = 0; ride && f < r->cfg.num_fields; ++f) ride = p.out[f] != out_fields[f];
  if (p.pending && !ride) {
    const hipStream_t old = p.st;
    const int rc = flush_pipe(r, p);
    if (rc != ACME_OK) return rc;
    if (old != st) {
      ACME_HIP_TRY(hipEventRecord(p.ev, old));
      ACME_HIP_TRY(hipStreamWaitEvent(st, p.ev, 0));
    }
  }
  if (!pair || 2 * nvec > 192 * kPipeChunks) {
    return sample_gather_impl(r, batch, step_counter, 1.0, slots, keys, probabilities,
                              table_size, priorities, out_fields, stream);
  }
  SampleTable t;
  int rc = sample_prologue(r, st, &t);
  if (rc != ACME_OK) return rc;
  const int64_t pend = ride ? p.batch : 0;
  SmallFields psm = {};
  uint8_t *pd0 = nullptr, *pd1 = nullptr;
  if (ride) {
    void* po[ACME_MAX_FIELDS];
    for (int f = 0; f < r->cfg.num_fields; ++f) po[f] = p.out[f];
    int g0, g1;
    pair_layout(r, po, &g0, &g1, &psm);
    pd0 = static_cast<uint8_t*>(po[g0]);
    pd1 = static_cast<uint8_t*>(po[g1]);
  }
  ACME_PROF("replay_sample_gather", st, 0.0,
            (double)batch * (40.0 + (t.prio ? 512.0 * r->nlevels : 0.0)) +
                (double)pend * 2.0 * row_bytes(r));
  const unsigned grid = (unsigned)std::max(batch, pend);
#define ACME_SGPIPE(PRIO)                                                                       \
  sample_gather_pipe_kernel<PRIO, kPipeChunks><<<grid, 256, 0, st>>>(                           \
      t.tv, r->raw_prio, r->keys, t.size, r->cfg.seed, step_counter, batch, slots, keys,        \
      probabilities, table_size, priorities, ride ? p.slots : nullptr, pend, r->fields[f0],     \
      r->fields[f1], pd0, pd1, nvec, psm)
  if (t.prio) ACME_SGPIPE(true);
  else ACME_SGPIPE(false);
#undef ACME_SGPIPE
  ACME_LAUNCH_CHECK();
  p.pending = true;
  p.st = st;
  p.batch = batch;
  p.slots = slots;
  for (int f = 0; f < ACME_MAX_FIELDS; ++f) p.out[f] = f < r->cfg.num_fields ? out_fields[f] : nullptr;
  return ACME_OK;
}

}

int acme::replay_update_priorities_gated(acme_replay* r, const uint64_t* keys,
                                         const double* prios, int64_t n, const Gate& gate,
                                         hipStream_t st, const RescaleJob* job) {
  ACME_CHECK_ARG(r && (n == 0 || (keys && prios)), "null argument");
  ACME_CHECK_ARG(n >= 0 && n < (int64_t(1) << 31), "bad update count");
  Gate eff = gate;
  if (n == 0 || n > kFusedUpdateMax) {
    if (job && job->s) {
      const int rc = launch_rescale_job(*job, st);
      if (rc != ACME_OK) return rc;
      if (job->rg.g && job->rg.mode == kRgStep) {
        eff = Gate{};
        eff.g = job->rg.g;
        eff.use_last = 1;
      }
    }
    if (n == 0) return ACME_OK;
  }
  std::lock_guard<std::mutex> lock(r->mu);
  int rc = order_after_inserts(r, st);
  if (rc != ACME_OK) return rc;
  if (n > r->upd_cap) {
    if (r->upd_slots) {
      ACME_HIP_TRY(hipDeviceSynchronize());
      (void)hipFree(r->upd_slots);
      (void)hipFree(r->upd_valid);
    }
    r->upd_cap = std::max<int64_t>(n, 4096);
    ACME_HIP_TRY(hipMalloc(&r->upd_slots, r->upd_cap * sizeof(int64_t)));
    ACME_HIP_TRY(hipMalloc(&r->upd_valid, r->upd_cap * sizeof(int32_t)));
  }
  int64_t* t_slots = r->upd_slots;
  int32_t* t_valid = r->upd_valid;
  const unsigned g = (unsigned)ceil_div(n, 256);
  const double alpha =
      r->cfg.sampler == ACME_SAMPLER_PRIORITIZED ? r->cfg.priority_exponent : 0.0;
  ACME_PROF("replay_update", st, 0.0, (double)n * (16.0 + 8.0 * 3 + 512.0 * (r->nlevels - 1)));
  if (n <= kFusedUpdateMax) {
    FusedUpdateArgs a;
    a.upd_keys = keys; a.prios = prios; a.n = (int)n; a.capacity = r->cfg.capacity;
    a.keys = r->keys; a.alpha = alpha; a.raw_prio = r->raw_prio; a.nlevels = r->nlevels;
    a.gate = gate;
    if (job) a.job = *job;
    for (int l = 0; l < 8; ++l) a.level[l] = r->levels[l];
    a.top_nodes = r->nlevels >= 2 ? r->level_size[r->nlevels - 2] / 64 : 0;
    a.top_computed = computed_top_nodes(r) > 0 ? 1 : 0;
    a.done = r->upd_done;
    a.stamps = g_update_stamps;
    const unsigned blocks = kFusedUpdateBlocks + (a.job.s ? 1 : 0);
    if (n <= 2 * 256) prio_update_fused_kernel<2><<<blocks, 256, 0, st>>>(a);
    else prio_update_fused_kernel<kFusedUpdateMax / 256><<<blocks, 256, 0, st>>>(a);
    ACME_LAUNCH_CHECK();
    return ACME_OK;
  }
  prio_resolve_kernel<<<g, 256, 0, st>>>(keys, n, r->keys, r->cfg.capacity, t_slots, t_valid,
                                         r->winner);
  ACME_LAUNCH_CHECK();
  prio_write_kernel<<<g, 256, 0, st>>>(prios, n, t_slots, t_valid, r->winner, alpha,
                                       r->raw_prio, r->levels[0], eff);
  ACME_LAUNCH_CHECK();
  for (int l = 1; l < r->nlevels; ++l) {
    level_update_kernel<<<(unsigned)ceil_div(n, 4), 256, 0, st>>>(
        r->levels[l - 1], r->levels[l], 0, n, t_slots, t_valid, 6 * l);
    ACME_LAUNCH_CHECK();
  }
  prio_reset_kernel<<<g, 256, 0, st>>>(t_slots, t_valid, n, r->winner);
  ACME_LAUNCH_CHECK();
  return ACME_OK;
}

extern "C" {

int acme_replay_update_priorities(acme_replay* r, const uint64_t* keys, const double* prios,
                                  int64_t n, void* stream) {
  return replay_update_priorities_gated(r, keys, prios, n, Gate{}, as_stream(stream));
}

int acme_replay_update_priorities_gated(acme_replay* r, const uint64_t* keys, const double* prios,
                                        int64_t n, const uint32_t* skip_word, void* stream) {
  Gate q;
  if (skip_word) {
    q.g = reinterpret_cast<const StepGuard*>(reinterpret_cast<const char*>(skip_word) -
                                             offsetof(StepGuard, last));
    q.use_last = 1;
  }
  return replay_update_priorities_gated(r, keys, prios, n, q, as_stream(stream));
}

}

struct acme_nstep_writer {
  acme_replay* r = nullptr;
  int n = 1;
  float g = 1.0f;
  int64_t obs_bytes = 0, act_bytes = 0;
  int64_t rows = 0;
  int64_t off[ACME_MAX_FIELDS + 3] = {};
  uint8_t* chunk[2] = {};
  uint8_t* mirror[2] = {};
  hipEvent_t done[2] = {}, up[2] = {};
  bool used[2] = {};
  int cur = 0;
  int64_t fill = 0;
  std::vector<double> prio;
  std::vector<uint8_t> obs, act;
  std::vector<float> rew, disc;
  int64_t lo = 0, steps = 0;
// ... 163 lines not shown
```

acme_amd/csrc/torso.h:

```cpp
#pragma once

#include <hip/hip_runtime.h>

#include <cstdint>

#include "conv.h"

namespace acme {
namespace gemm {
struct PScale;
}
namespace torso {

using G1 = conv::Geom<84, 84, 4, 21, 21, 32, 8, 8, 4, 2, 2>;
using G2 = conv::Geom<21, 21, 32, 11, 11, 64, 4, 4, 2, 1, 1>;
using G3 = conv::Geom<11, 11, 64, 11, 11, 64, 3, 3, 1, 1, 1>;
constexpr int kFlat = 11 * 11 * 64;
constexpr int kObsBytes = 84 * 84 * 4;
constexpr int kX1 = G1::OPIX * G1::CO;

struct Weights {
  const float *w1, *b1, *w2, *b2, *w3, *b3;
};
struct Grads {
  float *w1, *b1, *w2, *b2, *w3, *b3;
};
struct Acts {
  float *x1, *x2, *x3;
};

int64_t wgrad_slab_floats();

int forward(const Weights& w, bool u8, const void* obs_a, const void* obs_b, int split, int rows,
            const Acts& a, hipStream_t st);

int backward(const Weights& w, const Grads& g, bool u8, const void* obs, int rows, const Acts& a,
             const float* dz3, float* dz2, float* dz1, float* slab, hipStream_t st);

struct Plane {
  uint16_t* p;
  int64_t stride;
  gemm::PScale* sc;
};
struct PWeights {
  Plane w1, w2, w3;
  const float *b1, *b2, *b3;
};
extern uint64_t* g_stamps_conv[3];

struct PActs {
  Plane x1, x2, x3;
};
int64_t wgrad_slab_floats_p3();
struct Frames {
  const void* p;
  bool u8 = false;
  const void* p2 = nullptr;
  int split = 1 << 30;
  Frames rows_from(int r) const {
    if (!u8) return Frames{static_cast<const uint8_t*>(p) + (size_t)r * kObsBytes * 2};
    if (r >= split)
      return Frames{static_cast<const uint8_t*>(p2) + (size_t)(r - split) * kObsBytes, true};
    return Frames{static_cast<const uint8_t*>(p) + (size_t)r * kObsBytes, true, p2, split - r};
  }
};
int forward_p3(const PWeights& w, const Frames& frames, int rows, const PActs& a,
               hipStream_t st, int keep_x1 = -1, bool bk32 = false);
struct WgradSlab {
  const float* slab = nullptr;
  int splits = 0;
  int64_t wcount = 0, bcount = 0;
};
struct Side {
  hipStream_t side = nullptr;
  float* slab = nullptr;
  hipEvent_t e[3] = {nullptr, nullptr, nullptr};
  float* slab2 = nullptr;
  WgradSlab* defer = nullptr;
  int (*tail)(void* ctx, hipStream_t st) = nullptr;
  void* tail_ctx = nullptr;
  bool single_role = false;
  bool conv1_single = false;
  bool bk32 = false;
};
int backward_p3(const PWeights& w, const Grads& g, const Frames& frames, int rows,
                const PActs& a, const Plane& dz3, const Plane& dz2, const Plane& dz1, float* slab,
                hipStream_t st, const Side& side = Side());

}
}
```

acme_amd/csrc/torso.hip:

```cpp
#include "torso.h"

#include <algorithm>

#include "common.h"
#include "conv_p3.h"
#include "gemm.h"
#include "gemm_p3.h"
#include "gemm_p3i.h"
#include "gemm_p3s.h"
#include "gemm_p3c12.h"
#include "gemm_x6.h"
#include "kernels.h"
#include "launch.h"
#include "plane_guard.h"
#include "profiler.h"

namespace acme {
namespace torso {

using namespace acme::conv;
using acme::gemm::launch_gemm;

namespace {

constexpr int kConv1WgradSplits = 256, kConv2WgradSplits = 64, kConv3WgradSplits = 64;

template <class G, class In, int BM, int BN, int WM, int WN>
int conv_wgrad(const typename In::T* x, const float* dz, int rows, int splits, float* slab,
               float* dw, float* db, const char* name, const char* rname, hipStream_t st) {
  ConvWgrad<G, In> p;
  p.M = G::K; p.N = G::CO; p.K = rows * G::OPIX; p.k_chunk = chunk_for(p.K, splits);
  p.x = x; p.dz = dz; p.slab = slab;
  ACME_GEMM(name, BM, BN, WM, WN, 16, 1, p, splits);
  const int64_t count = (int64_t)(p.M + 1) * p.N;
  ACME_PROF(rname, st, 0.0, 4.0 * (double)(splits + 1) * (double)count);
  return launch_slab_reduce(slab, splits, count, dw, (int64_t)p.M * p.N, db, nullptr, 0, 0, st);
}

}

int64_t wgrad_slab_floats() {
  return std::max<int64_t>({(int64_t)kConv1WgradSplits * (G1::K + 1) * G1::CO,
                            (int64_t)kConv2WgradSplits * (G2::K + 1) * G2::CO,
                            (int64_t)kConv3WgradSplits * (G3::K + 1) * G3::CO});
}

int forward(const Weights& w, bool u8, const void* obs_a, const void* obs_b, int split, int rows,
            const Acts& a, hipStream_t st) {
  if (u8) {
    ConvFwd<G1, InU8> p;
    p.M = rows * G1::OPIX; p.N = G1::CO; p.K = G1::K; p.k_chunk = G1::K;
    p.x = static_cast<const uint8_t*>(obs_a); p.x2 = static_cast<const uint8_t*>(obs_b);
    p.split_b = split; p.w = w.w1; p.bias = w.b1; p.y = a.x1;
    ACME_GEMM("conv1_fwd", 128, 32, 4, 1, 16, 1, p, 1);
  } else {
    ConvFwd<G1, InF32> p;
    p.M = rows * G1::OPIX; p.N = G1::CO; p.K = G1::K; p.k_chunk = G1::K;
    p.x = static_cast<const float*>(obs_a); p.x2 = static_cast<const float*>(obs_b);
    p.split_b = split; p.w = w.w1; p.bias = w.b1; p.y = a.x1;
    ACME_GEMM("conv1_fwd", 128, 32, 4, 1, 16, 1, p, 1);
  }
  {
    ConvFwd<G2, InF32> p;
    p.M = rows * G2::OPIX; p.N = G2::CO; p.K = G2::K; p.k_chunk = G2::K;
    p.x = a.x1; p.x2 = a.x1; p.split_b = rows; p.w = w.w2; p.bias = w.b2; p.y = a.x2;
    ACME_GEMM("conv2_fwd", 128, 64, 2, 2, 16, 1, p, 1);
  }
// ... 60 lines not shown
constexpr int kBkConv3Dgrad = 128, kBkConv2Dgrad = 32;
constexpr int kBkFused1 = 32, kBkFused2 = 64;

inline PlaneSrc frames_src(const Frames& f, int rows) {
  return PlaneSrc{static_cast<const uint16_t*>(f.p), 0,
                  (int32_t)((f.u8 ? 1 : 2) * (int64_t)rows * G1::IPIX * G1::CI)};
}

template <bool U8>
int conv1_fwd_p3(const PWeights& w, const Frames& frames, int rows, const Planes& y,
                 hipStream_t st, bool bk32, uint64_t* stamps = nullptr) {
  P3ConvFwd<G1, 1, U8> p;
  p.stamps = stamps;
  p.M = rows * G1::OPIX; p.N = G1::CO; p.K = G1::K; p.k_chunk = G1::K;
  const int n1 = U8 ? std::min(rows, frames.split) : rows;
  p.a_src = frames_src(frames, n1); p.b_src = SRC(w.w1, G1::K * G1::CO);
  if (U8 && n1 < rows) {
    p.a_src2 = frames_src(frames.rows_from(n1), rows - n1);
    p.a_split = n1;
  }
  p.bias = w.b1; p.y = y;
  P3I_GEMM_BK("conv1_fwd", I1F, 1, 32, 7, 1, 2, kBkConv1, bk32, p, rows);
  return ACME_OK;
}

template <bool U8>
int conv12_fwd_p3(const PWeights& w, const Frames& frames, int rows, int nsep, const PActs& a,
                  hipStream_t st, bool bk32) {
  const int nf = rows - nsep;
  const Frames fr = frames.rows_from(nsep);
  if (U8 && fr.split < nf)
    return (set_error("the fused conv1 -> conv2 forward reads its frames from one buffer"),
            ACME_ERR_INVALID);
  P3ConvFwd<G1, 1, U8> p1;
  p1.M = nf * G1::OPIX; p1.N = G1::CO; p1.K = G1::K; p1.k_chunk = G1::K;
  p1.a_src = frames_src(fr, nf); p1.b_src = SRC(w.w1, G1::K * G1::CO);
  p1.bias = w.b1;
  p1.y = Planes{a.x1.p + (int64_t)nsep * kX1, a.x1.stride, a.x1.sc};
  P3ConvFwd<G2, gemm::kPlanes> p2;
  p2.M = nf * G2::OPIX; p2.N = G2::CO; p2.K = G2::K; p2.k_chunk = G2::K;
  p2.a_src = SRC(a.x1, (int64_t)rows * kX1); p2.b_src = SRC(w.w2, G2::K * G2::CO);
  p2.bias = w.b2;
  p2.y = Planes{a.x2.p + (int64_t)nsep * kFlat, a.x2.stride, a.x2.sc};
  const double fl = 2.0 * p1.M * p1.N * (double)p1.K + 2.0 * p2.M * p2.N * (double)p2.K;
  ACME_PROF_PEAK("conv12_fwd", st, fl, 0.0, gemm::p3_peak_tflops<decltype(p2)>());
  hipError_t e = bk32 ? gemm::launch_gemm_p3c12<32, 32>(p1, p2, nf, 0, st)
                      : gemm::launch_gemm_p3c12<kBkFused1, kBkFused2>(p1, p2, nf, 0, st);
  if (e != hipSuccess) return (set_error("gemm launch failed: %s", hipGetErrorString(e)), ACME_ERR_HIP);
  return ACME_OK;
}

template <bool U8>
int conv1_wgrad_p3(const Frames& frames, int rows, const Plane& dz1, float* slab, int splits,
                   bool single_role, P3ConvWgrad<G1, 1, U8>& p, hipStream_t st) {
  if (U8 && frames.split < rows)
    return (set_error("conv1's weight gradient reads its frames from one buffer"),
            ACME_ERR_INVALID);
  P3ConvWgrad<G1, 1, U8> q;
  q.M = G1::K; q.N = G1::CO; q.K = rows * G1::OPIX;
  q.k_chunk = chunk_for(q.K, splits);
  q.a_src = frames_src(frames, rows); q.b_src = SRC(dz1, (int64_t)rows * kX1);
  q.slab = slab;
  if (single_role) ACME_P3_GEMM("conv1_wgrad", 256, 32, 4, 1, 32, q, splits);
  else ACME_P3WS_GEMM("conv1_wgrad", 256, 32, 4, 1, 32, q, splits);
  p = q;
  return ACME_OK;
}

template <class P>
int p3_wgrad_reduce(const P& p, int splits, float* slab, float* dw, float* db, const char* rname,
                    hipStream_t st) {
  const int64_t count = (int64_t)(p.M + 1) * p.N;
  ACME_PROF(rname, st, 0.0, 4.0 * (double)(splits + 1) * (double)count);
  return launch_slab_reduce(slab, splits, count, dw, (int64_t)p.M * p.N, db, nullptr, 0, 0, st);
}

}

uint64_t* g_stamps_conv[3] = {nullptr, nullptr, nullptr};

int64_t wgrad_slab_floats_p3() {
  return std::max<int64_t>({(int64_t)kP3MaxWgradSplits * (G1::K + 1) * G1::CO,
                            (int64_t)kP3MaxWgradSplits * (G2::K + 1) * G2::CO,
                            (int64_t)kP3MaxWgradSplits * (G3::K + 1) * G3::CO});
}

int forward_p3(const PWeights& w, const Frames& frames, int rows, const PActs& a,
               hipStream_t st, int keep_x1, bool bk32) {
  const int nsep = keep_x1 == 0 ? 0 : rows;
  int rc;
  if (nsep < rows &&
      (rc = frames.u8 ? conv12_fwd_p3<true>(w, frames, rows, nsep, a, st, bk32)
                      : conv12_fwd_p3<false>(w, frames, rows, nsep, a, st, bk32)) != ACME_OK)
    return rc;
  if (nsep > 0 && (rc = frames.u8 ? conv1_fwd_p3<true>(w, frames, nsep, PP(a.x1), st, bk32, g_stamps_conv[0])
                                  : conv1_fwd_p3<false>(w, frames, nsep, PP(a.x1), st, bk32, g_stamps_conv[0])) != ACME_OK)
    return rc;
  if (nsep > 0) {
    P3ConvFwd<G2, gemm::kPlanes> p;
    p.M = nsep * G2::OPIX; p.N = G2::CO; p.K = G2::K; p.k_chunk = G2::K;
    p.a_src = SRC(a.x1, (int64_t)nsep * kX1); p.b_src = SRC(w.w2, G2::K * G2::CO);
    p.bias = w.b2; p.y = PP(a.x2);
    p.stamps = g_stamps_conv[1];
    P3I_GEMM_BK("conv2_fwd", I2F, 2, 64, 8, 2, 1, kBkConv2, bk32, p, nsep);
  }
  {
    P3ConvFwd<G3, gemm::kPlanes> p;
    p.M = rows * G3::OPIX; p.N = G3::CO; p.K = G3::K; p.k_chunk = G3::K;
    p.a_src = SRC(a.x2, (int64_t)rows * kFlat); p.b_src = SRC(w.w3, G3::K * G3::CO);
    p.bias = w.b3; p.y = PP(a.x3);
    if (keep_x1 != 0) p.stamps = g_stamps_conv[2];
    P3I_GEMM_BK("conv3_fwd", I3F, 1, 64, 4, 2, 1, kBkConv3, bk32, p, rows);
  }
  return ACME_OK;
}

// ... 13 lines not shown
      ACME_HIP_TRY(hipStreamWaitEvent(sd.side, sd.e[0], 0));
    }
    P3ConvWgrad<G3, gemm::kPlanes> p;
    p.M = G3::K; p.N = G3::CO; p.K = rows * G3::OPIX;
    const int splits = kP3Conv3WgradSplits;
    p.k_chunk = chunk_for(p.K, splits);
    p.a_src = SRC(a.x2, (int64_t)rows * kFlat); p.b_src = SRC(dz3, (int64_t)rows * kFlat);
    p.slab = wslab;
    ACME_P3_GEMM("conv3_wgrad", 128, 64, 2, 2, 32, p, splits);
    if (defer) sd.defer[2] = WgradSlab{wslab, splits, (int64_t)p.M * p.N, p.N};
    else if ((rc = p3_wgrad_reduce(p, splits, wslab, g.w3, g.b3, "conv3_wgrad_reduce", st)))
      return rc;
  }
  st = st_main;
  {
    P3ConvDgrad<G3> p;
    p.M = rows * G3::IPIX; p.N = G3::CI; p.K = G3::KH * G3::KW * G3::CO; p.k_chunk = p.K;
    p.a_src = SRC(dz3, (int64_t)rows * kFlat); p.b_src = SRC(w.w3, G3::K * G3::CO);
    p.xprev = CP(a.x2); p.dx = PP(dz2);
    P3I_GEMM_BK("conv3_dgrad", I3D, 2, 64, 8, 2, 1, kBkConv3Dgrad, sd.bk32, p, rows);
  }
  if (fork) {
    ACME_HIP_TRY(hipEventRecord(sd.e[1], st_main));
    ACME_HIP_TRY(hipStreamWaitEvent(sd.side, sd.e[1], 0));
    st = sd.side;
  }
  {
    P3ConvWgrad<G2, gemm::kPlanes> p;
    p.M = G2::K; p.N = G2::CO; p.K = rows * G2::OPIX;
    const int splits = kP3Conv2WgradSplits;
    p.k_chunk = chunk_for(p.K, splits);
    p.a_src = SRC(a.x1, (int64_t)rows * kX1); p.b_src = SRC(dz2, (int64_t)rows * kFlat);
    float* slab2 = defer ? sd.slab2 : wslab;
    p.slab = slab2;
    ACME_P3_GEMM("conv2_wgrad", 128, 64, 2, 2, 32, p, splits);
    if (defer) sd.defer[1] = WgradSlab{slab2, splits, (int64_t)p.M * p.N, p.N};
    else if ((rc = p3_wgrad_reduce(p, splits, slab2, g.w2, g.b2, "conv2_wgrad_reduce", st)))
      return rc;
    if (fork) ACME_HIP_TRY(hipEventRecord(sd.e[2], sd.side));
  }
  st = st_main;
  {
    P3ConvDgradSubZ<G2> p;
    p.M = P3ConvDgradSubZ<G2>::max_rows(rows); p.N = G2::CI; p.K = P3ConvDgradSubZ<G2>::KR;
    p.k_chunk = p.K; p.batch = rows;
    p.a_src = SRC(dz2, (int64_t)rows * kFlat); p.b_src = SRC(w.w2, G2::K * G2::CO);
    p.xprev = CP(a.x1); p.dx = PP(dz1);
    const double fl = 2.0 * rows * G2::IPIX * G2::CI * (double)p.K;
    ACME_PROF_PEAK("conv2_dgrad", st, fl, 0.0, gemm::p3_peak_tflops<decltype(p)>());
    hipError_t e = sd.bk32 ? gemm::launch_gemm_p3s<G2, 2, 32>(p, rows, st)
                           : gemm::launch_gemm_p3s<G2, 2, kBkConv2Dgrad>(p, rows, st);
    if (e != hipSuccess) return (set_error("gemm launch failed: %s", hipGetErrorString(e)), ACME_ERR_HIP);
  }
  {
    const int splits = kP3Conv1WgradSplits;
    int64_t wcount;
    int M1, N1;
    if (frames.u8) {
      P3ConvWgrad<G1, 1, true> p;
      if ((rc = conv1_wgrad_p3<true>(frames, rows, dz1, slab, splits, sd.conv1_single, p, st)))
        return rc;
      M1 = p.M, N1 = p.N;
      if (!defer && (rc = p3_wgrad_reduce(p, splits, slab, g.w1, g.b1, "conv1_wgrad_reduce", st)))
        return rc;
    } else {
      P3ConvWgrad<G1, 1> p;
      if ((rc = conv1_wgrad_p3<false>(frames, rows, dz1, slab, splits, sd.conv1_single, p, st)))
        return rc;
      M1 = p.M, N1 = p.N;
      if (!defer && (rc = p3_wgrad_reduce(p, splits, slab, g.w1, g.b1, "conv1_wgrad_reduce", st)))
        return rc;
    }
    wcount = (int64_t)M1 * N1;
    if (defer) sd.defer[0] = WgradSlab{slab, splits, wcount, N1};
  }
  if (sd.tail && (rc = sd.tail(sd.tail_ctx, st_main)) != ACME_OK) return rc;
  if (fork) ACME_HIP_TRY(hipStreamWaitEvent(st_main, sd.e[2], 0));
  return ACME_OK;
}

}
}
```

acme_amd/native.py:

```python

from __future__ import annotations

import ctypes
from typing import Dict, List, Optional, Sequence, Tuple

import numpy as np
import torch

from acme_amd import _lib
from acme_amd._lib import check, lib, ptr, stream_ptr

SAMPLER_UNIFORM = 0
SAMPLER_PRIORITIZED = 1


class NativeReplay:

    def __init__(self, capacity: int, field_bytes: Sequence[int], prioritized: bool,
                 priority_exponent: float = 0.6, seed: int = 1234, device=None):
        _lib.require_gpu()
        if len(field_bytes) > _lib.MAX_FIELDS:
            raise ValueError(f"at most {_lib.MAX_FIELDS} flattened fields per item")
        cfg = _lib.ReplayConfig()
        cfg.capacity = int(capacity)
# ... 133 lines not shown

    def export_state(self) -> Dict[str, np.ndarray]:
        L = lib()
        n = self.size()
        torch.cuda.synchronize(self.device)
        out = {"inserted": np.int64(L.acme_replay_inserted(self._h))}
        for f, b in enumerate(self.field_bytes):
            p = ctypes.c_void_p()
            check(L.acme_replay_storage(self._h, f, ctypes.byref(p)))
            out[f"field_{f}"] = _device_array(p.value, n * b, np.uint8, self.device).cpu() \
                .numpy().reshape(n, b).copy()
        lv, rp, ks = ctypes.c_void_p(), ctypes.c_void_p(), ctypes.c_void_p()
        check(L.acme_replay_debug_leaves(self._h, ctypes.byref(lv), ctypes.byref(rp),
                                         ctypes.byref(ks)))
        out["raw_priorities"] = _device_array(rp.value, n, np.float64, self.device).cpu() \
            .numpy().view(np.float64).copy()
        out["keys"] = _device_array(ks.value, n, np.uint64, self.device).cpu().numpy() \
            .view(np.uint64).copy()
        return out

    def import_state(self, state: Dict[str, np.ndarray]) -> None:
        L = lib()
        keys = np.asarray(state["keys"], np.uint64)
        n = len(keys)
        if n > self.capacity:
            raise ValueError(f"state holds {n} items, table capacity is {self.capacity}")
        torch.cuda.synchronize(self.device)
        for f, b in enumerate(self.field_bytes):
            rows = np.ascontiguousarray(state[f"field_{f}"], np.uint8)
            if rows.shape != (n, b):
                raise ValueError(f"field {f}: state rows {rows.shape}, table expects {(n, b)}")
            p = ctypes.c_void_p()
            check(L.acme_replay_storage(self._h, f, ctypes.byref(p)))
            _memcpy_htod(p.value, rows)
        lv, rp, ks = ctypes.c_void_p(), ctypes.c_void_p(), ctypes.c_void_p()
        check(L.acme_replay_debug_leaves(self._h, ctypes.byref(lv), ctypes.byref(rp),
                                         ctypes.byref(ks)))
        _memcpy_htod(rp.value, np.asarray(state["raw_priorities"], np.float64))
        _memcpy_htod(ks.value, keys)
        check(L.acme_replay_restore(self._h, int(state["inserted"]), None), "replay restore")
        torch.cuda.synchronize(self.device)

    def debug_state(self) -> Dict[str, np.ndarray]:
        lv, rp, ks = ctypes.c_void_p(), ctypes.c_void_p(), ctypes.c_void_p()
        check(lib().acme_replay_debug_leaves(self._h, ctypes.byref(lv), ctypes.byref(rp),
                                             ctypes.byref(ks)))
        torch.cuda.synchronize(self.device)
        n = self.capacity
        out = {}
        for name, p, dt, cnt in (("leaves", lv, np.float64, n), ("raw", rp, np.float64, n),
                                 ("keys", ks, np.uint64, n)):
            out[name] = _device_array(p.value, cnt, dt, self.device).cpu().numpy().view(dt).copy()
        return out


class NativeNStepWriter:

    def __init__(self, table: NativeReplay, n_step: int, discount: float, obs_bytes: int,
                 action_bytes: int, rows_per_chunk: int = 64):
        h = ctypes.c_void_p()
        L = lib()
        check(L.acme_nstep_writer_create(table.handle, int(n_step), float(discount),
                                         int(obs_bytes), int(action_bytes), int(rows_per_chunk),
                                         ctypes.byref(h)), "n-step writer create")
        self._table = table
        self._h = h
        self._add = L.acme_nstep_writer_add
        self._pending = L.acme_nstep_writer_pending

    def __del__(self):
        h = getattr(self, "_h", None)
        if h is not None and h.value:
            try:
                lib().acme_nstep_writer_destroy(h)
            except Exception:
                pass
            self._h = None

    def start(self, obs_ptr: int) -> None:
        check(lib().acme_nstep_writer_start(self._h, obs_ptr), "n-step writer start")

    def add_raw(self, act_ptr: int, reward: float, discount: float, obs_ptr: int, last: bool,
                priority: float = 1.0) -> None:
        rc = self._add(self._h, act_ptr, reward, discount, obs_ptr, 1 if last else 0, priority)
        if rc:
            check(rc, "n-step writer add")

    def flush(self) -> None:
        check(lib().acme_nstep_writer_flush(self._h), "n-step writer flush")

    def reset(self) -> None:
        check(lib().acme_nstep_writer_reset(self._h), "n-step writer reset")

    def pending(self) -> int:
        return int(self._pending(self._h))


def _device_array(address: int, count: int, dtype, device) -> torch.Tensor:
    nbytes = count * np.dtype(dtype).itemsize
    dst = torch.empty(nbytes, dtype=torch.uint8, device=device)
    torch.cuda.synchronize(device)
    _memcpy_dtod(dst.data_ptr(), address, nbytes)
    return dst


_hip = None
# ... 194 lines not shown
class NativeDQN(_PlaneState, _NativeLearner):

    _prefix, _tag = "acme_dqn", "dqn"
    plane_overflow = _plane_overflow

    def __init__(self, *, network: str, num_actions: int, max_batch: int, obs_dtype: str,
                 obs_dim: int = 0, hidden: Sequence[int] = (), discount: float = 0.99,
                 importance_sampling_exponent: float = 0.2, learning_rate: float = 1e-3,
                 huber_loss_parameter: float = 1.0, target_update_period: int = 100,
                 max_abs_reward: float = 1.0, adam_beta1: float = 0.9, adam_beta2: float = 0.999,
                 adam_epsilon: float = 1e-8, semantics: str = "tf", device=None):
        _lib.require_gpu()
        if semantics not in ("tf", "jax"):
            raise ValueError(f"semantics must be 'tf' or 'jax', got {semantics!r}")
        if huber_loss_parameter < 0:
            raise ValueError("quadratic_linear_boundary must be >= 0.")
        cfg = _lib.DQNConfig()
        cfg.network = NET_NATURE if network == "nature" else NET_MLP
        cfg.obs_dtype = OBS_U8 if obs_dtype == "uint8" else OBS_F32
        cfg.num_actions = int(num_actions)
        cfg.max_batch = int(max_batch)
        cfg.obs_dim = int(obs_dim)
        if len(hidden) > _lib.MAX_MLP_LAYERS:
            raise ValueError(f"at most {_lib.MAX_MLP_LAYERS} hidden layers")
        cfg.num_hidden = len(hidden)
        for i, h in enumerate(hidden):
            cfg.hidden[i] = int(h)
        cfg.discount = discount
        cfg.importance_sampling_exponent = importance_sampling_exponent
        cfg.learning_rate = learning_rate
        cfg.huber_loss_parameter = huber_loss_parameter
        cfg.adam_beta1, cfg.adam_beta2, cfg.adam_epsilon = adam_beta1, adam_beta2, adam_epsilon
        cfg.target_update_period = int(target_update_period)
        cfg.max_abs_reward = max_abs_reward
        cfg.semantics = _lib.SEMANTICS_JAX if semantics == "jax" else _lib.SEMANTICS_TF
        self.semantics = semantics
        self.network = network
        self.num_actions = int(num_actions)
        self.max_batch = int(max_batch)
        self._create(cfg, device)
        self.num_params = int(lib().acme_dqn_num_params(self._h))
        d = self.device
        self.loss = torch.zeros(1, dtype=torch.float32, device=d)
        self.td_error = torch.zeros(max_batch, dtype=torch.float32, device=d)
        self.priorities = torch.zeros(max_batch, dtype=torch.float64, device=d)

    def guard_state(self) -> Dict[str, int]:
        a = (ctypes.c_int64 * 4)()
        check(lib().acme_dqn_guard_state(self._h, a), "dqn guard_state")
        t = ctypes.c_int64()
        check(lib().acme_dqn_verdict_timeouts(self._h, ctypes.byref(t)), "dqn verdict_timeouts")
        return dict(applied=int(a[0]), skipped=int(a[1]), last_skipped=int(a[2]),
                    q_values_overflowed=int(a[3]), verdict_timeouts=int(t.value))

    @property
    def applied_steps(self) -> int:
        return self.guard_state()["applied"]

    @applied_steps.setter
    def applied_steps(self, n: int) -> None:
        check(lib().acme_dqn_set_applied_steps(self._h, int(n)), "dqn set_applied_steps")

    @property
    def skip_word(self) -> Optional[int]:
        p = ctypes.c_void_p()
        check(lib().acme_dqn_skip_word(self._h, ctypes.byref(p)), "dqn skip_word")
        return p.value

    def set_reissue(self, enable: bool) -> None:
        check(lib().acme_dqn_set_reissue(self._h, 1 if enable else 0), "dqn set_reissue")

    @property
    def verdicts_issued(self) -> int:
        return int(lib().acme_dqn_verdicts_issued(self._h))

    def step_verdict(self, seq: int) -> Optional[bool]:
        v = ctypes.c_int32(-1)
        check(lib().acme_dqn_step_verdict(self._h, int(seq), ctypes.byref(v)), "dqn step_verdict")
        return None if v.value < 0 else bool(v.value)

    def set_data_parallel_gate(self, enable: bool) -> None:
        check(lib().acme_dqn_set_data_parallel_gate(self._h, 1 if enable else 0), "dqn dp gate")

    def _batch(self, o_tm1, a_tm1, r_t, d_t, o_t, probabilities, global_min_probability=None,
               mean_over=None, obs_f16=None):
        B = int(a_tm1.shape[0])
        if B < 1 or B > self.max_batch:
            raise ValueError(f"batch of {B} rows: the learner takes 1..{self.max_batch}")
        for name, t in (("o_tm1", o_tm1), ("a_tm1", a_tm1), ("r_t", r_t), ("d_t", d_t),
                        ("o_t", o_t), ("probabilities", probabilities)):
            if not (isinstance(t, torch.Tensor) and t.is_cuda and t.is_contiguous()):
                raise ValueError(f"{name} must be a contiguous device tensor")
            if t.shape[0] != B:
                raise ValueError(f"{name} has leading dim {t.shape[0]}, expected {B}")
        if a_tm1.dtype != torch.int32 or r_t.dtype != torch.float32 or d_t.dtype != torch.float32:
            raise ValueError("a_tm1 must be int32, r_t and d_t float32")
        if probabilities.dtype != torch.float64:
            raise ValueError("probabilities must be float64")
        want = torch.uint8 if self.cfg.obs_dtype == OBS_U8 else torch.float32
        if o_tm1.dtype != want or o_t.dtype != want:
            raise ValueError(f"observations must be {want}")
        tb = _lib.TransitionBatch()
        tb.o_tm1, tb.a_tm1, tb.r_t, tb.d_t, tb.o_t = (ptr(o_tm1), ptr(a_tm1), ptr(r_t), ptr(d_t),
                                                      ptr(o_t))
        tb.probabilities = ptr(probabilities)
        tb.batch = B
# ... 499 lines not shown
```

include/acme_hip.h:

```cpp
#ifndef ACME_HIP_H_
#define ACME_HIP_H_

#include <stdint.h>

#ifdef __cplusplus
extern "C" {
#endif

typedef enum acme_status {
  ACME_OK = 0,
  ACME_ERR_INVALID = -1,
  ACME_ERR_HIP = -2,
  ACME_ERR_EMPTY = -3,
  ACME_ERR_OOM = -4
} acme_status;

const char* acme_last_error(void);

int acme_tune_set(const char* key, int32_t value);
const char* acme_version(void);
const char* acme_target_arch(void);

int acme_event_create(void** ev);
int acme_event_destroy(void* ev);
// ... 65 lines not shown
int acme_replay_gather(acme_replay* r, const int64_t* slots, int64_t batch,
                       void* const* out_fields, void* stream);

int acme_replay_sample_gather(acme_replay* r, int64_t batch, uint64_t step_counter,
                              int64_t* slots, uint64_t* keys, double* probabilities,
                              int64_t* table_size, double* priorities, void* const* out_fields,
                              void* stream);

int acme_replay_sample_gather_frames(acme_replay* r, int64_t batch, uint64_t step_counter,
                                     int64_t* slots, uint64_t* keys, double* probabilities,
                                     int64_t* table_size, double* priorities,
                                     void* const* out_fields, uint16_t* frames_f16,
                                     void* stream);

int acme_replay_pipe_open(acme_replay* r, int32_t* pipe);
int acme_replay_pipe_close(acme_replay* r, int32_t pipe);
int acme_replay_pipe_flush(acme_replay* r, int32_t pipe);
int acme_replay_sample_gather_pipe(acme_replay* r, int32_t pipe, int64_t batch,
                                   uint64_t step_counter, int64_t* slots, uint64_t* keys,
                                   double* probabilities, int64_t* table_size,
                                   double* priorities, void* const* out_fields, void* stream);

int acme_replay_total(acme_replay* r, double* out, void* stream);
int acme_replay_sample_share(acme_replay* r, int64_t batch, uint64_t step_counter,
                             double prob_scale, int64_t* slots, uint64_t* keys,
                             double* probabilities, int64_t* table_size, double* priorities,
                             void* const* out_fields, void* stream);
int acme_replay_sample_share_frames(acme_replay* r, int64_t batch, uint64_t step_counter,
                                    double prob_scale, int64_t* slots, uint64_t* keys,
                                    double* probabilities, int64_t* table_size,
                                    double* priorities, void* const* out_fields,
                                    uint16_t* frames_f16, void* stream);

int acme_frames_expand(const uint8_t* frames, int64_t num_frames, int64_t frame_bytes,
                       int32_t stack, const int32_t* idx, int64_t batch, uint8_t* out,
                       void* stream);

int acme_r2d2_priorities(const float* errors, int32_t T, int32_t B, double eta, double* out,
                         void* stream);
int acme_r2d2_importance_weights(const double* probabilities, int32_t B,
                                 int64_t max_replay_size, double beta, float* out,
                                 void* stream);

int acme_replay_update_priorities(acme_replay* r, const uint64_t* keys,
                                  const double* priorities, int64_t n, void* stream);
int acme_replay_update_priorities_gated(acme_replay* r, const uint64_t* keys,
                                        const double* priorities, int64_t n,
                                        const uint32_t* skip_word, void* stream);

int64_t acme_replay_size(const acme_replay* r);
int64_t acme_replay_capacity(const acme_replay* r);
int acme_replay_debug_leaves(const acme_replay* r, const double** leaf_values,
                             const double** raw_priorities, const uint64_t** keys);

int acme_replay_storage(acme_replay* r, int32_t field, void** out);
int64_t acme_replay_inserted(const acme_replay* r);
int acme_replay_restore(acme_replay* r, int64_t inserted, void* stream);


enum { ACME_NET_NATURE_DQN = 0, ACME_NET_MLP = 1 };
enum { ACME_SEMANTICS_TF = 0, ACME_SEMANTICS_JAX = 1 };
enum { ACME_OBS_U8_SCALED = 0, ACME_OBS_F32 = 1 };

#define ACME_MAX_MLP_LAYERS 8

typedef struct acme_dqn_config {
  int32_t network;
  int32_t obs_dtype;
  int32_t num_actions;
  int32_t max_batch;
  int32_t obs_dim;
  int32_t num_hidden;
  int32_t hidden[ACME_MAX_MLP_LAYERS];
  float discount;
  float importance_sampling_exponent;
  float learning_rate;
  float huber_loss_parameter;
  float adam_beta1, adam_beta2, adam_epsilon;
  int32_t target_update_period;
  float max_abs_reward;
  int32_t semantics;
} acme_dqn_config;

typedef struct acme_dqn acme_dqn;

int acme_dqn_create(const acme_dqn_config* cfg, acme_dqn** out);
int acme_dqn_destroy(acme_dqn* l);
int64_t acme_dqn_num_params(const acme_dqn* l);
int64_t acme_dqn_flat_size(const acme_dqn* l);
int32_t acme_dqn_num_tensors(const acme_dqn* l);
int acme_dqn_tensor_info(const acme_dqn* l, int32_t i, int64_t* offset, int64_t* numel,
                         int32_t* ndim, int64_t* shape4, const char** name);

int acme_dqn_bind(acme_dqn* l, float* params, float* target, float* grads, float* adam_m,
                  float* adam_v);
int acme_dqn_params_changed(acme_dqn* l);
int acme_dqn_plane_overflow(acme_dqn* l, int32_t* overflow, int32_t reset);
int64_t acme_dqn_skipped_steps(const acme_dqn* l);
int acme_dqn_guard_state(acme_dqn* l, int64_t* out4);
int acme_dqn_set_applied_steps(acme_dqn* l, int64_t n);
int acme_dqn_skip_word(const acme_dqn* l, const uint32_t** out);
int acme_dqn_set_data_parallel_gate(acme_dqn* l, int32_t enable);
int acme_dqn_set_reissue(acme_dqn* l, int32_t enable);
int acme_dqn_verdict_timeouts(acme_dqn* l, int64_t* out);
int64_t acme_dqn_verdicts_issued(const acme_dqn* l);
int acme_dqn_step_verdict(const acme_dqn* l, int64_t seq, int32_t* state);
int acme_dqn_scale_state(const acme_dqn* l, float* out, int32_t capacity, int32_t* count);
int acme_dqn_set_scale_state(acme_dqn* l, const float* in, int32_t count);

typedef struct acme_transition_batch {
  const void* o_tm1;
  const int32_t* a_tm1;
  const float* r_t;
  const float* d_t;
  const void* o_t;
  const double* probabilities;
  int64_t batch;
  const double* global_min_probability;
  int64_t mean_over;
  const uint16_t* obs_f16;
  void* inputs_event;
} acme_transition_batch;

typedef struct acme_dqn_outputs {
  float* loss;
  float* td_error;
  double* priorities;
  float* q_tm1;
} acme_dqn_outputs;

int acme_dqn_forward_backward(acme_dqn* l, const acme_transition_batch* batch,
                              const acme_dqn_outputs* out, void* stream);
int acme_dqn_forward_backward_stage(acme_dqn* l, const acme_transition_batch* batch,
                                    const acme_dqn_outputs* out, int32_t stage, void* stream);
int acme_dqn_grad_split(const acme_dqn* l, int64_t* split);
int acme_dqn_dense_grads_ready(acme_dqn* l, void* stream);
int acme_dqn_dp_init(acme_dqn* l, void* nccl_comm, int32_t world_size);
int acme_dqn_dp_step(acme_dqn* l, const acme_transition_batch* batch,
                     const acme_dqn_outputs* out, void* stream);
int acme_nccl_get_unique_id(uint8_t* out128);
int acme_nccl_comm_init(const uint8_t* id128, int32_t world_size, int32_t rank, void** comm);
int acme_nccl_comm_destroy(void* comm);
int acme_dqn_apply(acme_dqn* l, void* stream);
int acme_dqn_step(acme_dqn* l, const acme_transition_batch* batch,
                  const acme_dqn_outputs* out, void* stream);
int acme_dqn_step_update(acme_dqn* l, const acme_transition_batch* batch,
                         const acme_dqn_outputs* out, acme_replay* replay,
                         const uint64_t* keys, void* after_event, void* stream);
int acme_dqn_q_values(acme_dqn* l, const void* obs, int64_t batch, int32_t use_target,
                      float* q_out, void* stream);
int64_t acme_dqn_num_steps(const acme_dqn* l);
int acme_dqn_debug_buffer(const acme_dqn* l, const char* name, const float** out,
                          int64_t* count);
int acme_dqn_set_num_steps(acme_dqn* l, int64_t n);
int acme_min_f64(const double* x, int64_t n, double* out_dev, void* stream);

#define ACME_D4PG_MAX_LAYERS 4
#define ACME_D4PG_MAX_ACT 16
// ... 341 lines not shown
```

Before: 1.073 million transitions/s.

## Fuse prioritized-replay priority update into conv1 weight-gradient GEMM launch as rider blocks

Adds a rider mechanism where the replay priority sum-tree update runs as extra workgroups prepended to the conv1 weight-gradient GEMM kernel, sharing its LDS and launch. The separate update-tail kernel launch and its serialization on the main stream are meant to go away, and the small update work can overlap with GEMM tiles. In exchange it adds a combined kernel whose blocks compete with GEMM tiles, requires the single-role conv1 path, and adds prepare/release bookkeeping on the replay. It is enabled by default through a tune variant.

Result: faster. 1.085 million transitions/s, median of 6 (+1.1%).

```diff
diff --git a/acme_amd/_lib.py b/acme_amd/_lib.py
--- a/acme_amd/_lib.py
+++ b/acme_amd/_lib.py
@@ -224,6 +224,8 @@
     "acme_replay_capacity": (c_i64, [c_vp]),
     "acme_replay_debug_leaves": (c_i32, [c_vp, ctypes.POINTER(c_vp), ctypes.POINTER(c_vp),
                                          ctypes.POINTER(c_vp)]),
+    "acme_replay_debug_level": (c_i32, [c_vp, c_i32, ctypes.POINTER(c_vp),
+                                        ctypes.POINTER(c_i64), ctypes.POINTER(c_i32)]),
     "acme_replay_storage": (c_i32, [c_vp, c_i32, ctypes.POINTER(c_vp)]),
     "acme_replay_inserted": (c_i64, [c_vp]),
     "acme_replay_restore": (c_i32, [c_vp, c_i64, c_vp]),
@@ -241,6 +243,7 @@
     "acme_dqn_skipped_steps": (c_i64, [c_vp]),
     "acme_dqn_guard_state": (c_i32, [c_vp, ctypes.POINTER(c_i64)]),
     "acme_dqn_verdict_timeouts": (c_i32, [c_vp, ctypes.POINTER(c_i64)]),
+    "acme_dqn_update_rider_launches": (c_i64, [c_vp]),
     "acme_dqn_set_applied_steps": (c_i32, [c_vp, c_i64]),
     "acme_dqn_skip_word": (c_i32, [c_vp, ctypes.POINTER(c_vp)]),
     "acme_dqn_set_reissue": (c_i32, [c_vp, c_i32]),
diff --git a/acme_amd/csrc/common.h b/acme_amd/csrc/common.h
--- a/acme_amd/csrc/common.h
+++ b/acme_amd/csrc/common.h
@@ -12,7 +12,7 @@
 
 void set_error(const char* fmt, ...);
 
-int tune_variant(const char* key);
+int tune_variant(const char* key, int unset = 0);
 void tune_set(const char* key, int value);
 int tune_generation();
 
diff --git a/acme_amd/csrc/common.hip b/acme_amd/csrc/common.hip
--- a/acme_amd/csrc/common.hip
+++ b/acme_amd/csrc/common.hip
@@ -28,12 +28,12 @@
   return g_tune_gen;
 }
 
-int tune_variant(const char* key) {
+int tune_variant(const char* key, int unset) {
   std::lock_guard<std::mutex> lock(g_tune_mu);
   for (auto& kv : g_tune)
     if (kv.first == key) return kv.second;
   const char* v = getenv((std::string("ACME_V_") + key).c_str());
-  const int x = v ? atoi(v) : 0;
+  const int x = v ? atoi(v) : unset;
   g_tune.emplace_back(key, x);
   return x;
 }
diff --git a/acme_amd/csrc/dqn.hip b/acme_amd/csrc/dqn.hip
--- a/acme_amd/csrc/dqn.hip
+++ b/acme_amd/csrc/dqn.hip
@@ -17,6 +17,7 @@
 #include "launch.h"
 #include "learner_common.h"
 #include "plane_guard.h"
+#include "prio_update.h"
 #include "profiler.h"
 #include "rccl_dyn.h"
 #include "torso.h"
@@ -103,6 +104,10 @@
   bool single_stream = false;
   bool single_role = false;
   bool bk32 = false;
+  bool update_rider = true;
+  int rider_groups = kUpdateRiderBlocks;
+  acme_replay* rider_replay = nullptr;
+  int64_t rider_launches = 0;
   bool frames_u8 = true;
   int64_t seq = 0;
   uint32_t* host_verdicts = nullptr;
@@ -326,6 +331,30 @@
       replay_update_priorities_gated(r, l->upd_keys, l->upd_prio, l->upd_n, step_gate(l), st, &job);
   if (rc == ACME_OK) l->step_rescaled = true;
   return rc;
+}
+
+int priority_update_rider(void* ctx, hipStream_t st, FusedUpdateArgs* out, bool* armed) {
+  acme_dqn* l = static_cast<acme_dqn*>(ctx);
+  acme_replay* r = l->upd_replay;
+  *armed = false;
+  if (!r || !l->upd_prio || l->upd_n < 1 || l->upd_n > kUpdateRiderMax) return ACME_OK;
+  if (l->upd_after) ACME_HIP_TRY(hipStreamWaitEvent(st, l->upd_after, 0));
+  const RescaleJob job = step_rescale_job(l, true);
+  const int rc = replay_update_prepare(r, l->upd_keys, l->upd_prio, l->upd_n, step_gate(l), st,
+                                       &job, l->rider_groups, out);
+  if (rc != ACME_OK) return rc;
+  l->upd_replay = nullptr;
+  l->rider_replay = r;
+  l->rider_launches += 1;
+  l->step_rescaled = true;
+  *armed = true;
+  return ACME_OK;
+}
+
+void priority_update_rider_done(void* ctx) {
+  acme_dqn* l = static_cast<acme_dqn*>(ctx);
+  if (l->rider_replay) replay_update_release(l->rider_replay);
+  l->rider_replay = nullptr;
 }
 
 int nature_backward(acme_dqn* l, const void* o_tm1, int B, hipStream_t st_main,
@@ -525,6 +554,8 @@
   l->single_stream = tune_variant("SIDE") == 1;
   l->single_role = tune_variant("WSN") == 1;
   l->bk32 = tune_variant("BK32") == 1;
+  l->update_rider = tune_variant("UPDATE_RIDER", kUpdateRiderDefault) != 0;
+  l->rider_groups = std::clamp(tune_variant("RIDER_GROUPS", kUpdateRiderBlocks), 1, 1024);
   l->stamps_on = tune_variant("STAMPS") == 1;
   const int A = cfg->num_actions;
   const int B = cfg->max_batch;
@@ -740,6 +771,8 @@
   return ACME_OK;
 }
 
+int64_t acme_dqn_update_rider_launches(const acme_dqn* l) { return l ? l->rider_launches : 0; }
+
 int acme_dqn_set_reissue(acme_dqn* l, int32_t enable) {
   ACME_CHECK_ARG(l, "null learner");
   l->sticky = enable != 0 && l->p3_capable;
@@ -931,6 +964,10 @@
       if (l->upd_replay && l->upd_prio && !l->calibrating) {
         sd.tail = priority_update_tail;
         sd.tail_ctx = l;
+        if (l->update_rider && l->fused_step && !l->dp_gate) {
+          sd.tail_rider = priority_update_rider;
+          sd.tail_rider_done = priority_update_rider_done;
+        }
       }
       if (l->fused_step && !l->calibrating && l->slab2) {
         sd.slab = l->side_slab;
diff --git a/acme_amd/csrc/gemm_p3.h b/acme_amd/csrc/gemm_p3.h
--- a/acme_amd/csrc/gemm_p3.h
+++ b/acme_amd/csrc/gemm_p3.h
@@ -15,10 +15,8 @@
   int m0, n0, z;
 };
 template <int BM, int BN>
-__device__ __forceinline__ BlockPlace place_block(int M, int N, int n_major) {
-  const int tiles = gridDim.x;
-  const int total = tiles * gridDim.z;
-  const int orig = blockIdx.x + tiles * blockIdx.z;
+__device__ __forceinline__ BlockPlace place_block_at(int orig, int tiles, int total, int M, int N,
+                                                     int n_major) {
   const int xcd = orig & 7, q = total >> 3, r = total & 7;
   const int L = (xcd < r ? xcd * (q + 1) : r * (q + 1) + (xcd - r) * q) + (orig >> 3);
   const int z = L / tiles, t = L - z * tiles;
@@ -32,6 +30,12 @@
     nt = t - mt * tiles_n;
   }
   return BlockPlace{mt * BM, nt * BN, z};
+}
+template <int BM, int BN>
+__device__ __forceinline__ BlockPlace place_block(int M, int N, int n_major) {
+  const int tiles = gridDim.x;
+  return place_block_at<BM, BN>(blockIdx.x + tiles * blockIdx.z, tiles, tiles * gridDim.z, M, N,
+                                n_major);
 }
 template <class P>
 __device__ __forceinline__ P z_select_at(const P& p, int z) {
@@ -513,14 +517,13 @@
 };
 
 template <int BM, int BN, int WM, int WN, int BK, bool DEEP, class P>
-__global__ void __launch_bounds__(64 * WM * WN) gemm_p3_kernel(const P p_in, int n_major) {
+__device__ __forceinline__ void gemm_p3_block(const P& p_in, const BlockPlace& bp,
+                                              uint8_t* smem) {
   using C = P3Core<BM, BN, WM, WN, BK, P>;
   using PA = typename C::PA;
   using PB = typename C::PB;
   constexpr int NT = C::NT, NPA = C::NPA, NPB = C::NPB, STAGE = C::STAGE;
-  const BlockPlace bp = place_block<BM, BN>(p_in.M, p_in.N, n_major);
   const P p = z_select_at(p_in, bp.z);
-  extern __shared__ __attribute__((aligned(16))) uint8_t smem[];
 
   const int tid = threadIdx.x;
   const int lane = tid & 63, wave = tid >> 6;
@@ -650,6 +653,29 @@
     }
   }
   C::epilogue(p, smem, m0, n0, wave, wm, wn, lane, split, acc, do_colsum);
+}
+
+template <int BM, int BN, int WM, int WN, int BK, bool DEEP, class P>
+__global__ void __launch_bounds__(64 * WM * WN) gemm_p3_kernel(const P p_in, int n_major) {
+  extern __shared__ __attribute__((aligned(16))) uint8_t smem[];
+  gemm_p3_block<BM, BN, WM, WN, BK, DEEP, P>(
+      p_in, place_block<BM, BN>(p_in.M, p_in.N, n_major), smem);
+}
+
+template <int BM, int BN, int WM, int WN, int BK, bool DEEP, class P, class R>
+__global__ void __launch_bounds__(64 * WM * WN)
+    gemm_p3r_kernel(const P p_in, int n_major, int tiles, const typename R::Args ra) {
+  extern __shared__ __attribute__((aligned(16))) uint8_t smem[];
+  const int nr = R::blocks(ra);
+  if ((int)blockIdx.x < nr) {
+    R::run(ra, smem, (int)blockIdx.x);
+    return;
+  }
+  gemm_p3_block<BM, BN, WM, WN, BK, DEEP, P>(
+      p_in,
+      place_block_at<BM, BN>((int)blockIdx.x - nr, tiles, (int)gridDim.x - nr, p_in.M, p_in.N,
+                             n_major),
+      smem);
 }
 
 template <int BM, int BN, int WM, int WN, int BK, int STAGES, class P>
@@ -964,6 +990,24 @@
   return hipGetLastError();
 }
 
+template <int BM, int BN, int WM, int WN, int BK, class R, bool DEEP = true, class P>
+inline hipError_t launch_gemm_p3_rider(const P& p, int splits, const typename R::Args& ra,
+                                       hipStream_t st) {
+  using C = P3Core<BM, BN, WM, WN, BK, P>;
+  constexpr int STAGES_BYTES = 2 * C::STAGE;
+  constexpr int LDS = STAGES_BYTES > C::EPI_BYTES ? STAGES_BYTES : C::EPI_BYTES;
+  static_assert(LDS <= 160 * 1024, "two stages must fit the 160-KiB LDS of a CU");
+  static_assert(R::kLdsBytes <= LDS, "the rider runs in the GEMM's LDS");
+  static_assert(R::kThreads == C::NT, "the rider's workgroup size is the GEMM's");
+  static hipError_t attr = p3_set_lds(&gemm_p3r_kernel<BM, BN, WM, WN, BK, DEEP, P, R>, LDS);
+  if (attr != hipSuccess) return attr;
+  const int tiles = ((p.N + BN - 1) / BN) * ((p.M + BM - 1) / BM);
+  hipLaunchKernelGGL((gemm_p3r_kernel<BM, BN, WM, WN, BK, DEEP, P, R>),
+                     dim3(R::blocks(ra) + tiles * splits), dim3(C::NT), LDS, st, p,
+                     p3_n_major(p), tiles, ra);
+  return hipGetLastError();
+}
+
 template <int BM, int BN, int WM, int WN, int BK, bool PIPE = false, class P>
 inline hipError_t launch_gemm_p3ws(const P& p, int splits, hipStream_t st) {
   using C = P3Core<BM, BN, WM, WN, BK, P>;
diff --git a/acme_amd/csrc/prio_update.h b/acme_amd/csrc/prio_update.h
--- /dev/null
+++ b/acme_amd/csrc/prio_update.h
@@ -0,0 +1,342 @@
+#pragma once
+
+#include <hip/hip_runtime.h>
+
+#include <cstdint>
+
+#include "detmath.h"
+#include "kernels.h"
+#include "rescale.h"
+
+struct acme_replay;
+
+namespace acme {
+
+template <int Ctrl>
+__device__ __forceinline__ double dpp_f64(double x) {
+  const uint64_t u = __builtin_bit_cast(uint64_t, x);
+  const int lo = __builtin_amdgcn_mov_dpp((int)(uint32_t)u, Ctrl, 0xf, 0xf, false);
+  const int hi = __builtin_amdgcn_mov_dpp((int)(uint32_t)(u >> 32), Ctrl, 0xf, 0xf, false);
+  return __builtin_bit_cast(double, ((uint64_t)(uint32_t)hi << 32) | (uint32_t)lo);
+}
+__device__ __forceinline__ double wave_total64(double x) {
+  x = x + dpp_f64<0xB1>(x);
+  x = x + dpp_f64<0x4E>(x);
+  x = x + dpp_f64<0x141>(x);
+  x = x + dpp_f64<0x140>(x);
+  const uint64_t u = __builtin_bit_cast(uint64_t, x);
+  const int lo = __builtin_amdgcn_ds_swizzle((int)(uint32_t)u, 0x401F);
+  const int hi = __builtin_amdgcn_ds_swizzle((int)(uint32_t)(u >> 32), 0x401F);
+  x = x + __builtin_bit_cast(double, ((uint64_t)(uint32_t)hi << 32) | (uint32_t)lo);
+  const uint64_t v = __builtin_bit_cast(uint64_t, x);
+  const uint32_t a0 = __builtin_amdgcn_readlane((int)(uint32_t)v, 31);
+  const uint32_t a1 = __builtin_amdgcn_readlane((int)(uint32_t)(v >> 32), 31);
+  const uint32_t b0 = __builtin_amdgcn_readlane((int)(uint32_t)v, 63);
+  const uint32_t b1 = __builtin_amdgcn_readlane((int)(uint32_t)(v >> 32), 63);
+  return __builtin_bit_cast(double, ((uint64_t)a1 << 32) | a0) +
+         __builtin_bit_cast(double, ((uint64_t)b1 << 32) | b0);
+}
+
+constexpr int kFusedUpdateMax = 4096;
+constexpr int kFusedUpdateBlocks = 256;
+constexpr int kUpdPairs = 32;
+constexpr int kUpdateRiderMax = 2 * 256;
+constexpr int kUpdateRiderBlocks = 64;
+constexpr int kUpdateRiderDefault = 1;
+struct FusedUpdateArgs {
+  const uint64_t* upd_keys;
+  const double* prios;
+  int n;
+  int64_t capacity;
+  const uint64_t* keys;
+  double alpha;
+  double* raw_prio;
+  double* level[8];
+  int64_t top_nodes;
+  int top_computed;
+  int nlevels;
+  int groups = kFusedUpdateBlocks;
+  uint32_t* done;
+  Gate gate;
+  RescaleJob job;
+  uint64_t* stamps = nullptr;
+};
+__device__ __forceinline__ bool wait_verdict_skip(StepGuard* g, uint32_t seq, uint32_t first) {
+  __shared__ uint32_t s_v;
+  if (threadIdx.x == 0) {
+    uint32_t v = first;
+    for (int it = 0; it < (1 << 22) && (v >> 1) != (seq & 0x7fffffffu); ++it) {
+      __builtin_amdgcn_s_sleep(2);
+      v = __hip_atomic_load(&g->vseq, __ATOMIC_RELAXED, __HIP_MEMORY_SCOPE_AGENT);
+    }
+    const bool got = (v >> 1) == (seq & 0x7fffffffu);
+    if (!got) atomicAdd(&g->vtimeout, 1u);
+    s_v = got ? (v & 1u) : 1u;
+  }
+  __syncthreads();
+  return s_v != 0u;
+}
+__device__ __forceinline__ void lds_barrier() {
+  __builtin_amdgcn_fence(__ATOMIC_RELEASE, "workgroup", "local");
+  __builtin_amdgcn_s_barrier();
+  __builtin_amdgcn_fence(__ATOMIC_ACQUIRE, "workgroup", "local");
+}
+__device__ __forceinline__ void store_shared_level(double* p, double v) {
+  __hip_atomic_store(p, v, __ATOMIC_RELAXED, __HIP_MEMORY_SCOPE_AGENT);
+}
+
+template <int R>
+struct UpdLds {
+  static constexpr int kCh = 0;
+  static constexpr int kSlot = kCh + kUpdPairs * 64 * 8;
+  static constexpr int kNode = kSlot + R * 256 * 8;
+  static constexpr int kNk = kNode + kUpdPairs * 8;
+  static constexpr int kVal = kNk + kUpdPairs * 8;
+  static constexpr int kLvl = kVal + kUpdPairs * 8;
+  static constexpr int kCnt = kLvl + kUpdPairs * 4;
+  static constexpr int kBytes = kCnt + 16;
+};
+
+template <int R>
+__device__ __forceinline__ void prio_update_body(const FusedUpdateArgs& a, uint8_t* lds,
+                                                 const int wg, const int G) {
+  static_assert(R * 256 <= kFusedUpdateMax, "update capacity");
+  using L = UpdLds<R>;
+  double(*s_ch)[64] = reinterpret_cast<double(*)[64]>(lds + L::kCh);
+  int64_t* s_slot = reinterpret_cast<int64_t*>(lds + L::kSlot);
+  int64_t* s_node = reinterpret_cast<int64_t*>(lds + L::kNode);
+  int64_t* s_nk = reinterpret_cast<int64_t*>(lds + L::kNk);
+  double* s_val = reinterpret_cast<double*>(lds + L::kVal);
+  int* s_lvl = reinterpret_cast<int*>(lds + L::kLvl);
+  int* s_cnt = reinterpret_cast<int*>(lds + L::kCnt);
+  int &s_len = s_cnt[0], &s_np = s_cnt[1], &s_ovf = s_cnt[2], &s_last = s_cnt[3];
+  const int first = a.job.s ? 1 : 0;
+  auto stamp = [&](int ph) {
+    if (a.stamps && threadIdx.x == 0)
+      a.stamps[8 * (int64_t)wg + ph] = __builtin_amdgcn_s_memrealtime();
+  };
+  stamp(0);
+  if (a.job.s && wg == 0) {
+    rescale_block(a.job);
+    stamp(1);
+    return;
+  }
+  const bool verdict = a.job.s && a.job.rg.g && a.job.rg.mode == kRgStep;
+  const int tid = threadIdx.x, nt = blockDim.x;
+  const int lane = tid & 63, wave = tid >> 6, nw = nt >> 6;
+  const int bid = wg - first;
+  const int h = a.nlevels >= 2 ? a.nlevels - 2 : 0;
+  bool skip = !verdict && gate_skip(a.gate);
+  if (tid == 0) s_len = 0;
+  __syncthreads();
+  uint64_t kv[R];
+  double pr[R];
+  int64_t sl[R];
+  int my_e[R];
+#pragma unroll
+  for (int i = 0; i < R; ++i) {
+    my_e[i] = -1;
+    kv[i] = 0;
+    pr[i] = 0.0;
+    sl[i] = 0;
+  }
+  if (!skip) {
+#pragma unroll
+    for (int i = 0; i < R; ++i) {
+      if (i * nt >= a.n) break;
+      const int j = tid + i * nt;
+      const int jc = j < a.n ? j : a.n - 1;
+      kv[i] = a.upd_keys[jc];
+      pr[i] = a.prios[jc];
+    }
+#pragma unroll
+    for (int i = 0; i < R; ++i) {
+      if (i * nt >= a.n) break;
+      const int j = tid + i * nt;
+      const int64_t slot = (int64_t)(kv[i] % (uint64_t)a.capacity);
+      if (j < a.n && (int)((uint32_t)(slot >> (6 * h)) % (uint32_t)G) == bid) {
+        const int e = atomicAdd(&s_len, 1);
+        s_slot[e] = slot;
+        my_e[i] = e;
+        sl[i] = slot;
+      }
+    }
+  }
+  __syncthreads();
+  stamp(1);
+  const int len = s_len;
+  if (len > 0) {
+    if (tid == 0) {
+      s_np = 0;
+      s_ovf = 0;
+    }
+    __syncthreads();
+    for (int idx = tid; idx < h * len; idx += nt) {
+      const int l = 1 + idx / len, e = idx - (l - 1) * len;
+      const int64_t node = s_slot[e] >> (6 * l);
+      bool first = true;
+      for (int f = 0; f < e && first; ++f) first = (s_slot[f] >> (6 * l)) != node;
+      if (!first) continue;
+      const int q = atomicAdd(&s_np, 1);
+      if (q < kUpdPairs) {
+        s_lvl[q] = l;
+        s_node[q] = node;
+        s_nk[q] = (node << 3) | l;
+      } else {
+        s_ovf = 1;
+      }
+    }
+    __syncthreads();
+    if (tid == 0 && s_np > kUpdPairs) s_np = kUpdPairs;
+    __syncthreads();
+    stamp(2);
+    const int np = s_np;
+    const bool pre = !s_ovf;
+    uint64_t kt[R];
+#pragma unroll
+    for (int i = 0; i < R; ++i) {
+      if (i * nt >= a.n) break;
+      kt[i] = my_e[i] >= 0 ? a.keys[sl[i]] : 0;
+    }
+    if (pre) {
+      for (int q = wave; q < np; q += nw)
+        s_ch[q][lane] = a.level[s_lvl[q] - 1][s_node[q] * 64 + lane];
+    }
+    double leafv[R];
+#pragma unroll
+    for (int i = 0; i < R; ++i) {
+      if (i * nt >= a.n) break;
+      leafv[i] = 0.0;
+      if (my_e[i] >= 0) leafv[i] = det_pow_priority(pr[i], a.alpha);
+    }
+#pragma unroll
+    for (int i = 0; i < R; ++i) {
+      if (i * nt >= a.n) break;
+      if (my_e[i] >= 0)
+        s_slot[my_e[i]] = (sl[i] << 13) | ((kt[i] == kv[i] ? 1 : 0) << 12) | (tid + i * nt);
+    }
+    __syncthreads();
+    stamp(4);
+    uint32_t vfirst = 0;
+    if (verdict && tid == 0)
+      vfirst = __hip_atomic_load(&a.job.rg.g->vseq, __ATOMIC_RELAXED, __HIP_MEMORY_SCOPE_AGENT);
+    bool winv[R];
+#pragma unroll
+    for (int i = 0; i < R; ++i) winv[i] = false;
+#pragma unroll
+    for (int i = 0; i < R; ++i) {
+      if (i * nt >= a.n) break;
+      const int e = my_e[i];
+      bool win = e >= 0 && kt[i] == kv[i];
+      const int j = tid + i * nt;
+      const int64_t me = (sl[i] << 1) | 1;
+#pragma unroll 4
+      for (int f = 0; f < len; ++f) {
+        const int64_t x = s_slot[f];
+        if ((x >> 12) == me && (int)(x & 4095) > j) win = false;
+      }
+      winv[i] = win;
+    }
+    if (pre) {
+#pragma unroll
+      for (int i = 0; i < R; ++i) {
+        if (i * nt >= a.n) break;
+        if (!winv[i]) continue;
+        const int64_t k1 = ((sl[i] >> 6) << 3) | 1;
+#pragma unroll 4
+        for (int q = 0; q < np; ++q)
+          if (s_nk[q] == k1) s_ch[q][sl[i] & 63] = leafv[i];
+      }
+    }
+    lds_barrier();
+    if (pre) {
+      for (int l = 1; l <= h; ++l) {
+        for (int q = wave; q < np; q += nw) {
+          if (s_lvl[q] != l) continue;
+          const double v = wave_total64(s_ch[q][lane]);
+          if (lane == 63) s_val[q] = v;
+        }
+        lds_barrier();
+        if (tid < np && s_lvl[tid] == l) {
+          const int64_t kp = ((s_node[tid] >> 6) << 3) | (l + 1);
+#pragma unroll 4
+          for (int q = 0; q < np; ++q)
+            if (s_nk[q] == kp) s_ch[q][s_node[tid] & 63] = s_val[tid];
+        }
+        lds_barrier();
+      }
+    }
+    stamp(7);
+    if (verdict) skip = wait_verdict_skip(a.job.rg.g, a.job.rg.seq, vfirst);
+    stamp(3);
+    if (!skip) {
+#pragma unroll
+      for (int i = 0; i < R; ++i) {
+        if (i * nt >= a.n) break;
+        if (!winv[i]) continue;
+        a.raw_prio[sl[i]] = pr[i];
+        if (h == 0 && !a.top_computed) store_shared_level(a.level[0] + sl[i], leafv[i]);
+        else a.level[0][sl[i]] = leafv[i];
+      }
+      if (pre) {
+        for (int q = tid; q < np; q += nt) {
+          const int l = s_lvl[q];
+          if (l == h && !a.top_computed) store_shared_level(a.level[l] + s_node[q], s_val[q]);
+          else a.level[l][s_node[q]] = s_val[q];
+        }
+      } else {
+        __syncthreads();
+        for (int l = 1; l <= h; ++l) {
+          for (int e = wave; e < len; e += nw) {
+            const int64_t node = (s_slot[e] >> 13) >> (6 * l);
+            const double v = wave_total64(a.level[l - 1][node * 64 + lane]);
+            if (lane == 63) {
+              if (l == h && !a.top_computed) store_shared_level(a.level[l] + node, v);
+              else a.level[l][node] = v;
+            }
+          }
+          __syncthreads();
+        }
+      }
+      stamp(5);
+    }
+  }
+  stamp(6);
+  if (a.nlevels < 2 || a.top_computed) return;
+  __builtin_amdgcn_fence(__ATOMIC_RELEASE, "agent");
+  __syncthreads();
+  if (tid == 0)
+    s_last = __hip_atomic_fetch_add(a.done, 1u, __ATOMIC_ACQ_REL, __HIP_MEMORY_SCOPE_AGENT) ==
+             (uint32_t)(G - 1);
+  __syncthreads();
+  if (!s_last) return;
+  __builtin_amdgcn_fence(__ATOMIC_ACQUIRE, "agent");
+  const int top = a.nlevels - 1;
+  for (int64_t node = wave; node < a.top_nodes; node += nw) {
+    const double c = __hip_atomic_load(a.level[top - 1] + node * 64 + lane, __ATOMIC_RELAXED,
+                                       __HIP_MEMORY_SCOPE_AGENT);
+    const double v = wave_total64(c);
+    if (lane == 63) a.level[top][node] = v;
+  }
+  if (tid == 0) __hip_atomic_store(a.done, 0u, __ATOMIC_RELAXED, __HIP_MEMORY_SCOPE_AGENT);
+}
+
+struct UpdateRider {
+  using Args = FusedUpdateArgs;
+  static constexpr int kThreads = 256;
+  static constexpr int kLdsBytes = UpdLds<kUpdateRiderMax / 256>::kBytes;
+  static __host__ __device__ __forceinline__ int blocks(const Args& a) {
+    return (a.groups + (a.job.s ? 1 : 0) + 7) & ~7;
+  }
+  static __device__ __forceinline__ void run(const Args& a, uint8_t* lds, int wg) {
+    if (wg < a.groups + (a.job.s ? 1 : 0))
+      prio_update_body<kUpdateRiderMax / 256>(a, lds, wg, a.groups);
+  }
+};
+
+int replay_update_prepare(acme_replay* r, const uint64_t* keys, const double* prios, int64_t n,
+                          const Gate& gate, hipStream_t st, const RescaleJob* job, int groups,
+                          FusedUpdateArgs* out);
+void replay_update_release(acme_replay* r);
+
+}
diff --git a/acme_amd/csrc/replay.hip b/acme_amd/csrc/replay.hip
--- a/acme_amd/csrc/replay.hip
+++ b/acme_amd/csrc/replay.hip
@@ -11,6 +11,7 @@
 #include "common.h"
 #include "detmath.h"
 #include "kernels.h"
+#include "prio_update.h"
 #include "profiler.h"
 #include "rescale.h"
 
@@ -86,31 +87,6 @@
   return x;
 }
 
-template <int Ctrl>
-__device__ __forceinline__ double dpp_f64(double x) {
-  const uint64_t u = __builtin_bit_cast(uint64_t, x);
-  const int lo = __builtin_amdgcn_mov_dpp((int)(uint32_t)u, Ctrl, 0xf, 0xf, false);
-  const int hi = __builtin_amdgcn_mov_dpp((int)(uint32_t)(u >> 32), Ctrl, 0xf, 0xf, false);
-  return __builtin_bit_cast(double, ((uint64_t)(uint32_t)hi << 32) | (uint32_t)lo);
-}
-__device__ __forceinline__ double wave_total64(double x) {
-  x = x + dpp_f64<0xB1>(x);
-  x = x + dpp_f64<0x4E>(x);
-  x = x + dpp_f64<0x141>(x);
-  x = x + dpp_f64<0x140>(x);
-  const uint64_t u = __builtin_bit_cast(uint64_t, x);
-  const int lo = __builtin_amdgcn_ds_swizzle((int)(uint32_t)u, 0x401F);
-  const int hi = __builtin_amdgcn_ds_swizzle((int)(uint32_t)(u >> 32), 0x401F);
-  x = x + __builtin_bit_cast(double, ((uint64_t)(uint32_t)hi << 32) | (uint32_t)lo);
-  const uint64_t v = __builtin_bit_cast(uint64_t, x);
-  const uint32_t a0 = __builtin_amdgcn_readlane((int)(uint32_t)v, 31);
-  const uint32_t a1 = __builtin_amdgcn_readlane((int)(uint32_t)(v >> 32), 31);
-  const uint32_t b0 = __builtin_amdgcn_readlane((int)(uint32_t)v, 63);
-  const uint32_t b1 = __builtin_amdgcn_readlane((int)(uint32_t)(v >> 32), 63);
-  return __builtin_bit_cast(double, ((uint64_t)a1 << 32) | a0) +
-         __builtin_bit_cast(double, ((uint64_t)b1 << 32) | b0);
-}
-
 __device__ __forceinline__ int select_child(double v, double s, double t) {
   const uint64_t le = __ballot(s <= t);
   const uint64_t nz = __ballot(v > 0.0);
@@ -601,271 +577,11 @@
   winner[slots[j]] = -1;
 }
 
-constexpr int kFusedUpdateMax = 4096;
-constexpr int kFusedUpdateBlocks = 256;
-constexpr int kUpdPairs = 32;
-struct FusedUpdateArgs {
-  const uint64_t* upd_keys;
-  const double* prios;
-  int n;
-  int64_t capacity;
-  const uint64_t* keys;
-  double alpha;
-  double* raw_prio;
-  double* level[8];
-  int64_t top_nodes;
-  int top_computed;
-  int nlevels;
-  uint32_t* done;
-  Gate gate;
-  RescaleJob job;
-  uint64_t* stamps = nullptr;
-};
-__device__ __forceinline__ bool wait_verdict_skip(StepGuard* g, uint32_t seq, uint32_t first) {
-  __shared__ uint32_t s_v;
-  if (threadIdx.x == 0) {
-    uint32_t v = first;
-    for (int it = 0; it < (1 << 22) && (v >> 1) != (seq & 0x7fffffffu); ++it) {
-      __builtin_amdgcn_s_sleep(2);
-      v = __hip_atomic_load(&g->vseq, __ATOMIC_RELAXED, __HIP_MEMORY_SCOPE_AGENT);
-    }
-    const bool got = (v >> 1) == (seq & 0x7fffffffu);
-    if (!got) atomicAdd(&g->vtimeout, 1u);
-    s_v = got ? (v & 1u) : 1u;
-  }
-  __syncthreads();
-  return s_v != 0u;
-}
-__device__ __forceinline__ void lds_barrier() {
-  __builtin_amdgcn_fence(__ATOMIC_RELEASE, "workgroup", "local");
-  __builtin_amdgcn_s_barrier();
-  __builtin_amdgcn_fence(__ATOMIC_ACQUIRE, "workgroup", "local");
-}
-__device__ __forceinline__ void store_shared_level(double* p, double v) {
-  __hip_atomic_store(p, v, __ATOMIC_RELAXED, __HIP_MEMORY_SCOPE_AGENT);
-}
 template <int R>
 __global__ void __launch_bounds__(256) prio_update_fused_kernel(FusedUpdateArgs a) {
-  static_assert(R * 256 <= kFusedUpdateMax, "update capacity");
-  __shared__ int64_t s_slot[R * 256];
-  __shared__ int s_len, s_np, s_ovf, s_last;
-  __shared__ double s_ch[kUpdPairs][64];
-  __shared__ int64_t s_node[kUpdPairs];
-  __shared__ int s_lvl[kUpdPairs];
-  __shared__ int64_t s_nk[kUpdPairs];
-  __shared__ double s_val[kUpdPairs];
-  const int first = a.job.s ? 1 : 0;
-  auto stamp = [&](int ph) {
-    if (a.stamps && threadIdx.x == 0)
-      a.stamps[8 * (int64_t)blockIdx.x + ph] = __builtin_amdgcn_s_memrealtime();
-  };
-  stamp(0);
-  if (a.job.s && blockIdx.x == 0) {
-    rescale_block(a.job);
-    stamp(1);
-    return;
-  }
-  const bool verdict = a.job.s && a.job.rg.g && a.job.rg.mode == kRgStep;
-  const int tid = threadIdx.x, nt = blockDim.x;
-  const int lane = tid & 63, wave = tid >> 6, nw = nt >> 6;
-  const int G = kFusedUpdateBlocks, bid = (int)blockIdx.x - first;
-  const int h = a.nlevels >= 2 ? a.nlevels - 2 : 0;
-  bool skip = !verdict && gate_skip(a.gate);
-  if (tid == 0) s_len = 0;
-  __syncthreads();
-  uint64_t kv[R];
-  double pr[R];
-  int64_t sl[R];
-  int my_e[R];
-#pragma unroll
-  for (int i = 0; i < R; ++i) {
-    my_e[i] = -1;
-    kv[i] = 0;
-    pr[i] = 0.0;
-    sl[i] = 0;
-  }
-  if (!skip) {
-#pragma unroll
-    for (int i = 0; i < R; ++i) {
-      if (i * nt >= a.n) break;
-      const int j = tid + i * nt;
-      const int jc = j < a.n ? j : a.n - 1;
-      kv[i] = a.upd_keys[jc];
-      pr[i] = a.prios[jc];
-    }
-#pragma unroll
-    for (int i = 0; i < R; ++i) {
-      if (i * nt >= a.n) break;
-      const int j = tid + i * nt;
-      const int64_t slot = (int64_t)(kv[i] % (uint64_t)a.capacity);
-      if (j < a.n && (int)((slot >> (6 * h)) % G) == bid) {
-        const int e = atomicAdd(&s_len, 1);
-        s_slot[e] = slot;
-        my_e[i] = e;
-        sl[i] = slot;
-      }
-    }
-  }
-  __syncthreads();
-  stamp(1);
-  const int len = s_len;
-  if (len > 0) {
-    if (tid == 0) {
-      s_np = 0;
-      s_ovf = 0;
-    }
-    __syncthreads();
-    for (int idx = tid; idx < h * len; idx += nt) {
-      const int l = 1 + idx / len, e = idx - (l - 1) * len;
-      const int64_t node = s_slot[e] >> (6 * l);
-      bool first = true;
-      for (int f = 0; f < e && first; ++f) first = (s_slot[f] >> (6 * l)) != node;
-      if (!first) continue;
-      const int q = atomicAdd(&s_np, 1);
-      if (q < kUpdPairs) {
-        s_lvl[q] = l;
-        s_node[q] = node;
-        s_nk[q] = (node << 3) | l;
-      } else {
-        s_ovf = 1;
-      }
-    }
-    __syncthreads();
-    if (tid == 0 && s_np > kUpdPairs) s_np = kUpdPairs;
-    __syncthreads();
-    stamp(2);
-    const int np = s_np;
-    const bool pre = !s_ovf;
-    uint64_t kt[R];
-#pragma unroll
-    for (int i = 0; i < R; ++i) {
-      if (i * nt >= a.n) break;
-      kt[i] = my_e[i] >= 0 ? a.keys[sl[i]] : 0;
-    }
-    if (pre) {
-      for (int q = wave; q < np; q += nw)
-        s_ch[q][lane] = a.level[s_lvl[q] - 1][s_node[q] * 64 + lane];
-    }
-    double leafv[R];
-#pragma unroll
-    for (int i = 0; i < R; ++i) {
-      if (i * nt >= a.n) break;
-      leafv[i] = 0.0;
-      if (my_e[i] >= 0) leafv[i] = det_pow_priority(pr[i], a.alpha);
-    }
-#pragma unroll
-    for (int i = 0; i < R; ++i) {
-      if (i * nt >= a.n) break;
-      if (my_e[i] >= 0)
-        s_slot[my_e[i]] = (sl[i] << 13) | ((kt[i] == kv[i] ? 1 : 0) << 12) | (tid + i * nt);
-    }
-    __syncthreads();
-    stamp(4);
-    uint32_t vfirst = 0;
-    if (verdict && tid == 0)
-      vfirst = __hip_atomic_load(&a.job.rg.g->vseq, __ATOMIC_RELAXED, __HIP_MEMORY_SCOPE_AGENT);
-    bool winv[R];
-#pragma unroll
-    for (int i = 0; i < R; ++i) winv[i] = false;
-#pragma unroll
-    for (int i = 0; i < R; ++i) {
-      if (i * nt >= a.n) break;
-      const int e = my_e[i];
-      bool win = e >= 0 && kt[i] == kv[i];
-      const int j = tid + i * nt;
-      const int64_t me = (sl[i] << 1) | 1;
-#pragma unroll 4
-      for (int f = 0; f < len; ++f) {
-        const int64_t x = s_slot[f];
-        if ((x >> 12) == me && (int)(x & 4095) > j) win = false;
-      }
-      winv[i] = win;
-    }
-    if (pre) {
-#pragma unroll
-      for (int i = 0; i < R; ++i) {
-        if (i * nt >= a.n) break;
-        if (!winv[i]) continue;
-        const int64_t k1 = ((sl[i] >> 6) << 3) | 1;
-#pragma unroll 4
-        for (int q = 0; q < np; ++q)
-          if (s_nk[q] == k1) s_ch[q][sl[i] & 63] = leafv[i];
-      }
-    }
-    lds_barrier();
-    if (pre) {
-      for (int l = 1; l <= h; ++l) {
-        for (int q = wave; q < np; q += nw) {
-          if (s_lvl[q] != l) continue;
-          const double v = wave_total64(s_ch[q][lane]);
-          if (lane == 63) s_val[q] = v;
-        }
-        lds_barrier();
-        if (tid < np && s_lvl[tid] == l) {
-          const int64_t kp = ((s_node[tid] >> 6) << 3) | (l + 1);
-#pragma unroll 4
-          for (int q = 0; q < np; ++q)
-            if (s_nk[q] == kp) s_ch[q][s_node[tid] & 63] = s_val[tid];
-        }
-        lds_barrier();
-      }
-    }
-    stamp(7);
-    if (verdict) skip = wait_verdict_skip(a.job.rg.g, a.job.rg.seq, vfirst);
-    stamp(3);
-    if (!skip) {
-#pragma unroll
-      for (int i = 0; i < R; ++i) {
-        if (i * nt >= a.n) break;
-        if (!winv[i]) continue;
-        a.raw_prio[sl[i]] = pr[i];
-        if (h == 0 && !a.top_computed) store_shared_level(a.level[0] + sl[i], leafv[i]);
-        else a.level[0][sl[i]] = leafv[i];
-      }
-      if (pre) {
-        for (int q = tid; q < np; q += nt) {
-          const int l = s_lvl[q];
-          if (l == h && !a.top_computed) store_shared_level(a.level[l] + s_node[q], s_val[q]);
-          else a.level[l][s_node[q]] = s_val[q];
-        }
-      } else {
-        __syncthreads();
-        for (int l = 1; l <= h; ++l) {
-          for (int e = wave; e < len; e += nw) {
-            const int64_t node = (s_slot[e] >> 13) >> (6 * l);
-            const double v = wave_total64(a.level[l - 1][node * 64 + lane]);
-            if (lane == 63) {
-              if (l == h && !a.top_computed) store_shared_level(a.level[l] + node, v);
-              else a.level[l][node] = v;
-            }
-          }
-          __syncthreads();
-        }
-      }
-      stamp(5);
-    }
-  }
-  stamp(6);
-  if (a.nlevels < 2 || a.top_computed) return;
-  __builtin_amdgcn_fence(__ATOMIC_RELEASE, "agent");
-  __syncthreads();
-  if (tid == 0)
-    s_last = __hip_atomic_fetch_add(a.done, 1u, __ATOMIC_ACQ_REL, __HIP_MEMORY_SCOPE_AGENT) ==
-             (uint32_t)(G - 1);
-  __syncthreads();
-  if (!s_last) return;
-  __builtin_amdgcn_fence(__ATOMIC_ACQUIRE, "agent");
-  const int top = a.nlevels - 1;
-  for (int64_t node = wave; node < a.top_nodes; node += nw) {
-    const double c = __hip_atomic_load(a.level[top - 1] + node * 64 + lane, __ATOMIC_RELAXED,
-                                       __HIP_MEMORY_SCOPE_AGENT);
-    const double v = wave_total64(c);
-    if (lane == 63) a.level[top][node] = v;
-  }
-  if (tid == 0) __hip_atomic_store(a.done, 0u, __ATOMIC_RELAXED, __HIP_MEMORY_SCOPE_AGENT);
-}
-
-
+  __shared__ __attribute__((aligned(16))) uint8_t s_mem[UpdLds<R>::kBytes];
+  prio_update_body<R>(a, s_mem, (int)blockIdx.x, a.groups);
+}
 
 __global__ void fill_i32_kernel(int32_t* p, int64_t n, int32_t v) {
   const int64_t i = (int64_t)blockIdx.x * blockDim.x + threadIdx.x;
@@ -1337,6 +1053,16 @@
   if (leaf_values) *leaf_values = r->levels[0];
   if (raw_priorities) *raw_priorities = r->raw_prio;
   if (keys) *keys = r->keys;
+  return ACME_OK;
+}
+
+int acme_replay_debug_level(const acme_replay* r, int32_t level, const double** values,
+                            int64_t* count, int32_t* nlevels) {
+  ACME_CHECK_ARG(r, "null replay");
+  if (nlevels) *nlevels = r->nlevels;
+  ACME_CHECK_ARG(level >= 0 && level < r->nlevels, "level %d out of range", level);
+  if (values) *values = r->levels[level];
+  if (count) *count = r->level_size[level];
   return ACME_OK;
 }
 
@@ -1935,6 +1661,50 @@
 
 }
 
+namespace {
+int update_scratch(acme_replay* r, int64_t n) {
+  if (n > r->upd_cap) {
+    if (r->upd_slots) {
+      ACME_HIP_TRY(hipDeviceSynchronize());
+      (void)hipFree(r->upd_slots);
+      (void)hipFree(r->upd_valid);
+    }
+    r->upd_cap = std::max<int64_t>(n, 4096);
+    ACME_HIP_TRY(hipMalloc(&r->upd_slots, r->upd_cap * sizeof(int64_t)));
+    ACME_HIP_TRY(hipMalloc(&r->upd_valid, r->upd_cap * sizeof(int32_t)));
+  }
+  return ACME_OK;
+}
+}
+
+int acme::replay_update_prepare(acme_replay* r, const uint64_t* keys, const double* prios,
+                                int64_t n, const Gate& gate, hipStream_t st,
+                                const RescaleJob* job, int groups, FusedUpdateArgs* out) {
+  ACME_CHECK_ARG(r && keys && prios && out, "null argument");
+  ACME_CHECK_ARG(n >= 1 && n <= kFusedUpdateMax && groups >= 1, "bad update or workgroup count");
+  std::unique_lock<std::mutex> lock(r->mu);
+  int rc = order_after_inserts(r, st);
+  if (rc != ACME_OK) return rc;
+  if ((rc = update_scratch(r, n)) != ACME_OK) return rc;
+  FusedUpdateArgs a;
+  a.upd_keys = keys; a.prios = prios; a.n = (int)n; a.capacity = r->cfg.capacity;
+  a.keys = r->keys; a.raw_prio = r->raw_prio; a.nlevels = r->nlevels;
+  a.alpha = r->cfg.sampler == ACME_SAMPLER_PRIORITIZED ? r->cfg.priority_exponent : 0.0;
+  a.gate = gate;
+  if (job) a.job = *job;
+  for (int l = 0; l < 8; ++l) a.level[l] = r->levels[l];
+  a.top_nodes = r->nlevels >= 2 ? r->level_size[r->nlevels - 2] / 64 : 0;
+  a.top_computed = computed_top_nodes(r) > 0 ? 1 : 0;
+  a.groups = groups;
+  a.done = r->upd_done;
+  a.stamps = g_update_stamps;
+  *out = a;
+  lock.release();
+  return ACME_OK;
+}
+
+void acme::replay_update_release(acme_replay* r) { r->mu.unlock(); }
+
 int acme::replay_update_priorities_gated(acme_replay* r, const uint64_t* keys,
                                          const double* prios, int64_t n, const Gate& gate,
                                          hipStream_t st, const RescaleJob* job) {
@@ -1953,42 +1723,30 @@
     }
     if (n == 0) return ACME_OK;
   }
+  if (n <= kFusedUpdateMax) {
+    const int tg = tune_variant("UPD_GROUPS");
+    FusedUpdateArgs a;
+    const int rc = replay_update_prepare(r, keys, prios, n, gate, st, job,
+                                         tg >= 1 && tg <= 1024 ? tg : kFusedUpdateBlocks, &a);
+    if (rc != ACME_OK) return rc;
+    std::lock_guard<std::mutex> lock(r->mu, std::adopt_lock);
+    ACME_PROF("replay_update", st, 0.0, (double)n * (16.0 + 8.0 * 3 + 512.0 * (r->nlevels - 1)));
+    const unsigned blocks = a.groups + (a.job.s ? 1 : 0);
+    if (n <= 2 * 256) prio_update_fused_kernel<2><<<blocks, 256, 0, st>>>(a);
+    else prio_update_fused_kernel<kFusedUpdateMax / 256><<<blocks, 256, 0, st>>>(a);
+    ACME_LAUNCH_CHECK();
+    return ACME_OK;
+  }
   std::lock_guard<std::mutex> lock(r->mu);
   int rc = order_after_inserts(r, st);
   if (rc != ACME_OK) return rc;
-  if (n > r->upd_cap) {
-    if (r->upd_slots) {
-      ACME_HIP_TRY(hipDeviceSynchronize());
-      (void)hipFree(r->upd_slots);
-      (void)hipFree(r->upd_valid);
-    }
-    r->upd_cap = std::max<int64_t>(n, 4096);
-    ACME_HIP_TRY(hipMalloc(&r->upd_slots, r->upd_cap * sizeof(int64_t)));
-    ACME_HIP_TRY(hipMalloc(&r->upd_valid, r->upd_cap * sizeof(int32_t)));
-  }
+  if ((rc = update_scratch(r, n)) != ACME_OK) return rc;
   int64_t* t_slots = r->upd_slots;
   int32_t* t_valid = r->upd_valid;
   const unsigned g = (unsigned)ceil_div(n, 256);
   const double alpha =
       r->cfg.sampler == ACME_SAMPLER_PRIORITIZED ? r->cfg.priority_exponent : 0.0;
   ACME_PROF("replay_update", st, 0.0, (double)n * (16.0 + 8.0 * 3 + 512.0 * (r->nlevels - 1)));
-  if (n <= kFusedUpdateMax) {
-    FusedUpdateArgs a;
-    a.upd_keys = keys; a.prios = prios; a.n = (int)n; a.capacity = r->cfg.capacity;
-    a.keys = r->keys; a.alpha = alpha; a.raw_prio = r->raw_prio; a.nlevels = r->nlevels;
-    a.gate = gate;
-    if (job) a.job = *job;
-    for (int l = 0; l < 8; ++l) a.level[l] = r->levels[l];
-    a.top_nodes = r->nlevels >= 2 ? r->level_size[r->nlevels - 2] / 64 : 0;
-    a.top_computed = computed_top_nodes(r) > 0 ? 1 : 0;
-    a.done = r->upd_done;
-    a.stamps = g_update_stamps;
-    const unsigned blocks = kFusedUpdateBlocks + (a.job.s ? 1 : 0);
-    if (n <= 2 * 256) prio_update_fused_kernel<2><<<blocks, 256, 0, st>>>(a);
-    else prio_update_fused_kernel<kFusedUpdateMax / 256><<<blocks, 256, 0, st>>>(a);
-    ACME_LAUNCH_CHECK();
-    return ACME_OK;
-  }
   prio_resolve_kernel<<<g, 256, 0, st>>>(keys, n, r->keys, r->cfg.capacity, t_slots, t_valid,
                                          r->winner);
   ACME_LAUNCH_CHECK();
diff --git a/acme_amd/csrc/torso.h b/acme_amd/csrc/torso.h
--- a/acme_amd/csrc/torso.h
+++ b/acme_amd/csrc/torso.h
@@ -7,6 +7,7 @@
 #include "conv.h"
 
 namespace acme {
+struct FusedUpdateArgs;
 namespace gemm {
 struct PScale;
 }
@@ -79,6 +80,8 @@
   WgradSlab* defer = nullptr;
   int (*tail)(void* ctx, hipStream_t st) = nullptr;
   void* tail_ctx = nullptr;
+  int (*tail_rider)(void* ctx, hipStream_t st, FusedUpdateArgs* out, bool* armed) = nullptr;
+  void (*tail_rider_done)(void* ctx) = nullptr;
   bool single_role = false;
   bool conv1_single = false;
   bool bk32 = false;
diff --git a/acme_amd/csrc/torso.hip b/acme_amd/csrc/torso.hip
--- a/acme_amd/csrc/torso.hip
+++ b/acme_amd/csrc/torso.hip
@@ -13,6 +13,7 @@
 #include "kernels.h"
 #include "launch.h"
 #include "plane_guard.h"
+#include "prio_update.h"
 #include "profiler.h"
 
 namespace acme {
@@ -179,7 +180,8 @@
 
 template <bool U8>
 int conv1_wgrad_p3(const Frames& frames, int rows, const Plane& dz1, float* slab, int splits,
-                   bool single_role, P3ConvWgrad<G1, 1, U8>& p, hipStream_t st) {
+                   bool single_role, P3ConvWgrad<G1, 1, U8>& p, hipStream_t st,
+                   const FusedUpdateArgs* rider = nullptr) {
   if (U8 && frames.split < rows)
     return (set_error("conv1's weight gradient reads its frames from one buffer"),
             ACME_ERR_INVALID);
@@ -188,7 +190,13 @@
   q.k_chunk = chunk_for(q.K, splits);
   q.a_src = frames_src(frames, rows); q.b_src = SRC(dz1, (int64_t)rows * kX1);
   q.slab = slab;
-  if (single_role) ACME_P3_GEMM("conv1_wgrad", 256, 32, 4, 1, 32, q, splits);
+  if (rider && !single_role)
+    return (set_error("the update rider needs conv1's single-role kernel"), ACME_ERR_INVALID);
+  if (rider)
+    ACME_LAUNCH_GEMM("conv1_wgrad", ACME_MNK_FLOPS(q), gemm::p3_peak_tflops<decltype(q)>(),
+                     (gemm::launch_gemm_p3_rider<256, 32, 4, 1, 32, UpdateRider>(q, splits, *rider,
+                                                                                 st)));
+  else if (single_role) ACME_P3_GEMM("conv1_wgrad", 256, 32, 4, 1, 32, q, splits);
   else ACME_P3WS_GEMM("conv1_wgrad", 256, 32, 4, 1, 32, q, splits);
   p = q;
   return ACME_OK;
@@ -308,21 +316,29 @@
                            : gemm::launch_gemm_p3s<G2, 2, kBkConv2Dgrad>(p, rows, st);
     if (e != hipSuccess) return (set_error("gemm launch failed: %s", hipGetErrorString(e)), ACME_ERR_HIP);
   }
+  FusedUpdateArgs upd;
+  bool rider = false;
+  if (sd.tail && sd.tail_rider && sd.tail_rider_done && sd.conv1_single &&
+      (rc = sd.tail_rider(sd.tail_ctx, st_main, &upd, &rider)) != ACME_OK)
+    return rc;
+  const FusedUpdateArgs* ride = rider ? &upd : nullptr;
   {
     const int splits = kP3Conv1WgradSplits;
     int64_t wcount;
     int M1, N1;
     if (frames.u8) {
       P3ConvWgrad<G1, 1, true> p;
-      if ((rc = conv1_wgrad_p3<true>(frames, rows, dz1, slab, splits, sd.conv1_single, p, st)))
-        return rc;
+      rc = conv1_wgrad_p3<true>(frames, rows, dz1, slab, splits, sd.conv1_single, p, st, ride);
+      if (rider) sd.tail_rider_done(sd.tail_ctx);
+      if (rc) return rc;
       M1 = p.M, N1 = p.N;
       if (!defer && (rc = p3_wgrad_reduce(p, splits, slab, g.w1, g.b1, "conv1_wgrad_reduce", st)))
         return rc;
     } else {
       P3ConvWgrad<G1, 1> p;
-      if ((rc = conv1_wgrad_p3<false>(frames, rows, dz1, slab, splits, sd.conv1_single, p, st)))
-        return rc;
+      rc = conv1_wgrad_p3<false>(frames, rows, dz1, slab, splits, sd.conv1_single, p, st, ride);
+      if (rider) sd.tail_rider_done(sd.tail_ctx);
+      if (rc) return rc;
       M1 = p.M, N1 = p.N;
       if (!defer && (rc = p3_wgrad_reduce(p, splits, slab, g.w1, g.b1, "conv1_wgrad_reduce", st)))
         return rc;
@@ -330,7 +346,7 @@
     wcount = (int64_t)M1 * N1;
     if (defer) sd.defer[0] = WgradSlab{slab, splits, wcount, N1};
   }
-  if (sd.tail && (rc = sd.tail(sd.tail_ctx, st_main)) != ACME_OK) return rc;
+  if (sd.tail && !rider && (rc = sd.tail(sd.tail_ctx, st_main)) != ACME_OK) return rc;
   if (fork) ACME_HIP_TRY(hipStreamWaitEvent(st_main, sd.e[2], 0));
   return ACME_OK;
 }
diff --git a/acme_amd/native.py b/acme_amd/native.py
--- a/acme_amd/native.py
+++ b/acme_amd/native.py
@@ -209,6 +209,21 @@
                                  ("keys", ks, np.uint64, n)):
             out[name] = _device_array(p.value, cnt, dt, self.device).cpu().numpy().view(dt).copy()
         return out
+
+    def debug_levels(self) -> list:
+        n = ctypes.c_int32()
+        p, cnt = ctypes.c_void_p(), ctypes.c_int64()
+        check(lib().acme_replay_debug_level(self._h, 0, ctypes.byref(p), ctypes.byref(cnt),
+                                            ctypes.byref(n)))
+        torch.cuda.synchronize(self.device)
+        out = []
+        for l in range(n.value):
+            check(lib().acme_replay_debug_level(self._h, l, ctypes.byref(p), ctypes.byref(cnt),
+                                                None))
+            out.append(_device_array(p.value, cnt.value, np.float64, self.device)
+                       .cpu().numpy().view(np.float64).copy())
+        return out
+
 
 
 class NativeNStepWriter:
@@ -509,6 +524,9 @@
         check(lib().acme_dqn_verdict_timeouts(self._h, ctypes.byref(t)), "dqn verdict_timeouts")
         return dict(applied=int(a[0]), skipped=int(a[1]), last_skipped=int(a[2]),
                     q_values_overflowed=int(a[3]), verdict_timeouts=int(t.value))
+
+    def update_rider_launches(self) -> int:
+        return int(lib().acme_dqn_update_rider_launches(self._h))
 
     @property
     def applied_steps(self) -> int:
diff --git a/include/acme_hip.h b/include/acme_hip.h
--- a/include/acme_hip.h
+++ b/include/acme_hip.h
@@ -141,6 +141,8 @@
 int64_t acme_replay_capacity(const acme_replay* r);
 int acme_replay_debug_leaves(const acme_replay* r, const double** leaf_values,
                              const double** raw_priorities, const uint64_t** keys);
+int acme_replay_debug_level(const acme_replay* r, int32_t level, const double** values,
+                            int64_t* count, int32_t* nlevels);
 
 int acme_replay_storage(acme_replay* r, int32_t field, void** out);
 int64_t acme_replay_inserted(const acme_replay* r);
@@ -193,6 +195,7 @@
 int acme_dqn_set_reissue(acme_dqn* l, int32_t enable);
 int acme_dqn_verdict_timeouts(acme_dqn* l, int64_t* out);
 int64_t acme_dqn_verdicts_issued(const acme_dqn* l);
+int64_t acme_dqn_update_rider_launches(const acme_dqn* l);
 int acme_dqn_step_verdict(const acme_dqn* l, int64_t seq, int32_t* state);
 int acme_dqn_scale_state(const acme_dqn* l, float* out, int32_t capacity, int32_t* count);
 int acme_dqn_set_scale_state(acme_dqn* l, const float* in, int32_t count);
```
